# gt1/daccord

Measured on AMD Instinct MI355X. Metric: corrected Mbase/s (whole node), synthetic 20x PacBio piles, higher is better.
Workload: dtype u64+f64

## Files before the change

daccord_amd/csrc/fast_diag.hpp:

```cpp
#ifndef DACC_FAST_DIAG_HPP
#define DACC_FAST_DIAG_HPP
#if defined(DACC_EMUL)
#include <cstdint>
#include <cstdio>
#include <cstdlib>
#include <vector>
#include <algorithm>
#endif

namespace dacc {

#if defined(DACC_EMUL)
struct FastStats { enum { N = 33 }; uint32_t v[N]; void clear() { for ( int i = 0; i < N; ++i ) v[i] = 0; } void mx(int i, uint32_t x) { if ( x > v[i] ) v[i] = x; } void add(int i, uint32_t x) { v[i] += x; } };
static FastStats g_fstats;
static inline void fstats_dump(int const tier)
{
	static FILE * sf = 0; static bool tried = false;
	if ( !tried ) { tried = true; char const * fn = getenv("DACC_EMUL_STATS"); if ( fn ) sf = fopen(fn,"w"); }
	if ( sf ) { fprintf(sf,"%d",tier); for ( int i = 0; i < FastStats::N; ++i ) fprintf(sf," %u",g_fstats.v[i]); fprintf(sf,"\n"); fflush(sf); }
}
static inline FILE * ftrav_file() { static FILE * f = 0; static bool tried = false; if ( !tried ) { tried = true; char const * fn = getenv("DACC_EMUL_TRAV"); if ( fn ) f = fopen(fn,"w"); } return f; }
#define FSTAT_MX(i,x) g_fstats.mx(i,x)
#define FSTAT_ADD(i,x) g_fstats.add(i,x)
struct FeasIters { std::vector<uint32_t> it, ln; void clear() { it.clear(); ln.clear(); } };
static FeasIters g_feasit;
static inline void feasit_dump()
{
	static FILE * f = 0; static bool tried = false;
	if ( !tried ) { tried = true; char const * fn = getenv("DACC_EMUL_FEAS"); if ( fn ) f = fopen(fn,"w"); }
	if ( !f ) { g_feasit.clear(); return; }
	std::vector<uint32_t> const & it = g_feasit.it; std::vector<uint32_t> const & ln = g_feasit.ln;
	uint64_t tot = 0, lock = 0, locksorted = 0;
	for ( size_t i = 0; i < it.size(); ++i ) tot += it[i];
	for ( size_t i = 0; i < it.size(); i += 64 ) { uint32_t m = 0; for ( size_t q = i; q < it.size() && q < i+64; ++q ) m = std::max(m,it[q]); lock += m; }
	std::vector< std::pair<uint32_t,uint32_t> > P; for ( size_t i = 0; i < it.size(); ++i ) P.push_back(std::make_pair(ln[i],it[i]));
	std::stable_sort(P.begin(),P.end(),[](std::pair<uint32_t,uint32_t> const & a, std::pair<uint32_t,uint32_t> const & b){ return a.first > b.first; });
	for ( size_t i = 0; i < P.size(); i += 64 ) { uint32_t m = 0; for ( size_t q = i; q < P.size() && q < i+64; ++q ) m = std::max(m,P[q].second); locksorted += m; }
	uint64_t lockcls = 0;
	{
		std::vector< std::pair<uint32_t,uint32_t> > Q; for ( size_t i = 0; i < it.size(); ++i ) { uint32_t c = 0; while ( (2u<<c) <= ln[i] ) ++c; Q.push_back(std::make_pair(c,it[i])); }
		std::stable_sort(Q.begin(),Q.end(),[](std::pair<uint32_t,uint32_t> const & a, std::pair<uint32_t,uint32_t> const & b){ return a.first > b.first; });
		for ( size_t i = 0; i < Q.size(); i += 64 ) { uint32_t m = 0; for ( size_t q = i; q < Q.size() && q < i+64; ++q ) m = std::max(m,Q[q].second); lockcls += m; }
	}
	fprintf(f,"%zu %llu %llu %llu %llu\n",it.size(),(unsigned long long)tot,(unsigned long long)lock,(unsigned long long)locksorted,(unsigned long long)lockcls);
	g_feasit.clear();
}
static inline bool feasit_on() { static int on = -1; if ( on < 0 ) on = getenv("DACC_EMUL_FEAS") ? 1 : 0; return on == 1; }
#define FEAS_ITERS(t,len,n) { if ( feasit_on() && !feascount ) { g_feasit.it.push_back(n); g_feasit.ln.push_back(len); } }
#define FEAS_DUMP() { if ( feasit_on() && !feascount ) feasit_dump(); }
struct FeasCases
{
	enum { NU = 0, NCU, NTASK, EMPTY_FIRST, EMPTY_MID, EMPTY_LAST, START_AT_ROUND, START_AT_ROUND_END, SPANS_ROUNDS, ROUNDS, LENMASK, MAXLEN, AT_CLAMP, PAST_CLAMP, MULTI, FAIL0, FAIL1, FAILLAST, NODES, N };
	uint64_t v[N];
	void clear() { for ( int i = 0; i < N; ++i ) v[i] = 0; }
	template<typename PT> void units(PT W, uint32_t const nu)
	{
		clear();
		v[NU] = nu;
		uint32_t first = nu, last = 0;
		for ( uint32_t q = 0; q < nu; ++q ) if ( W[q] ) { if ( first == nu ) first = q; last = q; }
		uint64_t t = 0;
		for ( uint32_t q = 0; q < nu; ++q )
		{
			uint32_t const w = W[q];
			if ( !w ) { if ( q < first ) ++v[EMPTY_FIRST]; else if ( q > last ) ++v[EMPTY_LAST]; else ++v[EMPTY_MID]; continue; }
			++v[NCU];
			if ( t && t % 64 == 0 ) ++v[START_AT_ROUND];
			if ( t % 64 == 63 ) ++v[START_AT_ROUND_END];
			if ( t/64 != (t+w-1)/64 ) ++v[SPANS_ROUNDS];
			t += w;
		}
		v[NTASK] = t; v[ROUNDS] = (t+63)/64;
	}
	void node(uint32_t const j, uint32_t const len, uint32_t const pp, uint32_t const nrows, uint32_t const f)
	{
		++v[NODES];
		if ( j == 0 ) { v[LENMASK] |= 1ull << (len < 63 ? len : 63); if ( len > v[MAXLEN] ) v[MAXLEN] = len; }
		if ( pp+1 == nrows ) ++v[AT_CLAMP];
		if ( pp >= nrows ) ++v[PAST_CLAMP];
		if ( f > 1 ) ++v[MULTI];
	}
	void fail(uint32_t const j, uint32_t const len) { if ( j == 0 ) ++v[FAIL0]; if ( j == 1 ) ++v[FAIL1]; if ( j+1 == len && len > 2 ) ++v[FAILLAST]; }
	void dump(int const tier, uint32_t const nwF, uint32_t const nwR)
	{
		static FILE * f = 0; static bool tried = false;
		if ( !tried ) { tried = true; char const * fn = getenv("DACC_EMUL_FEASCASES"); if ( fn ) f = fopen(fn,"w"); }
		if ( !f ) return;
		fprintf(f,"%d",tier); for ( int i = 0; i < N; ++i ) fprintf(f," %llu",(unsigned long long)v[i]); fprintf(f," %u %u\n",nwF,nwR); fflush(f);
	}
};
static FeasCases g_feascases;
#define FEAS_UNITS(W,nu) { if ( lane == 0 && !feascount ) g_feascases.units(W,nu); }
#define FEAS_NODE(j,len,pp,nrows,f) { if ( !feascount ) g_feascases.node(j,len,pp,nrows,f); }
#define FEAS_FAIL(j,len) { if ( !feascount ) g_feascases.fail(j,len); }
#define FEAS_CASES_DUMP() { if ( lane == 0 && !feascount ) g_feascases.dump(int(CT::maxs),nwF,nwR); }
struct FeasNeedAudit
{
	enum { SCAP = 65536 };
	uint64_t outF[SCAP][3], outR[SCAP][3];
	uint64_t ntrav, units0, tasks0, units1, tasks1, recF, recR, probeF, probeR, linkR, insF, insL, mids, hlek, passes;
	FILE * f; bool tried;
	bool on() { if ( !tried ) { tried = true; char const * fn = getenv("DACC_EMUL_FEASNEED"); if ( fn ) f = fopen(fn,"w"); } return f != 0; }
	static void range(uint64_t * m, uint32_t const lo, uint32_t const hi) { for ( uint32_t p = lo; p < hi && p < 192u; ++p ) m[p>>6] |= 1ull << (p&63u); }
	void unit(uint32_t const s, bool const rev, uint32_t const lo0, uint32_t const hi0, uint32_t const lo1, uint32_t const hi1)
	{
		if ( !on() || s >= SCAP ) return;
		uint64_t * const m = rev ? outR[s] : outF[s];
		m[0] = m[1] = m[2] = 0; range(m,lo0,hi0);
		uint64_t k[3] = {0,0,0}; range(k,lo1,hi1); m[0] &= ~k[0]; m[1] &= ~k[1]; m[2] &= ~k[2];
		if ( hi0 > lo0 ) { ++units0; tasks0 += hi0-lo0; }
		if ( hi1 > lo1 ) { ++units1; tasks1 += hi1-lo1; }
	}
	static bool out(uint64_t const * m, uint32_t const p) { return p < 192u && ((m[p>>6] >> (p&63u)) & 1ull); }
	void probe(uint32_t const s, bool const rev, uint32_t const p) { if ( f && s < SCAP && out(rev ? outR[s] : outF[s],p) ) ++(rev ? probeR : probeF); }
	void link(uint32_t const a, uint32_t const b) { if ( f && a < SCAP && b < SCAP && ((outR[a][0]|outR[a][1]|outR[a][2]) || (outR[b][0]|outR[b][1]|outR[b][2])) ) ++linkR; }
	void dump()
	{
		if ( !f ) return;
		rewind(f);
		fprintf(f,"%llu %llu %llu %llu %llu %llu %llu %llu %llu %llu %llu %llu %llu %llu %llu\n",(unsigned long long)ntrav,(unsigned long long)units0,(unsigned long long)tasks0,(unsigned long long)units1,(unsigned long long)tasks1,
			(unsigned long long)recF,(unsigned long long)recR,(unsigned long long)probeF,(unsigned long long)probeR,(unsigned long long)linkR,
			(unsigned long long)insF,(unsigned long long)insL,(unsigned long long)mids,(unsigned long long)hlek,(unsigned long long)passes);
		fflush(f);
	}
	~FeasNeedAudit() { dump(); }
};
static FeasNeedAudit g_feasneed;
#define FEAS_NEED_UNIT(s,rev,lo0,hi0,lo1,hi1) { if ( !feascount ) g_feasneed.unit(s,rev,lo0,hi0,lo1,hi1); }
#define FEAS_NEED_PROBE(s,rev,p) g_feasneed.probe(s,rev,p);
#define FEAS_NEED_LINK(a,b) g_feasneed.link(a,b);
#define FEAS_OVER() { if ( !feascount ) over(128); }
#define FEAS_NEED_PASS() { if ( lane == 0 ) ++g_feasneed.passes; }
#define FEAS_NEED_DUMP() { if ( lane == 0 && !feascount && g_feasneed.on() ) { FeasNeedAudit & A_ = g_feasneed; ++A_.ntrav; A_.recF += nwF; A_.recR += nwR; A_.mids += nmid; A_.hlek += (H <= static_cast<int64_t>(k)); \
	for ( uint32_t c_ = 0; c_ < nF; ++c_ ) A_.insF += (L.fnode()[c_] != 0xFFFF && L.parF()[c_] != SNONE); for ( uint32_t c_ = 0; c_ < nL; ++c_ ) A_.insL += (L.lnode()[c_] != 0xFFFF && L.parL()[c_] != SNONE); A_.dump(); } }
#else
#define FEAS_ITERS(t,len,n)
#define FEAS_DUMP()
#define FEAS_UNITS(W,nu)
#define FEAS_NODE(j,len,pp,nrows,f)
#define FEAS_FAIL(j,len)
#define FEAS_CASES_DUMP()
#define FEAS_NEED_UNIT(s,rev,lo0,hi0,lo1,hi1)
#define FEAS_NEED_PROBE(s,rev,p)
#define FEAS_NEED_LINK(a,b)
#define FEAS_NEED_DUMP()
#define FEAS_NEED_PASS()
#define FEAS_OVER() over(128);
#define FSTAT_MX(i,x)
#define FSTAT_ADD(i,x)
#endif
}
#endif
```

daccord_amd/csrc/fast_layout.hpp:

```cpp
#ifndef DACC_FAST_LAYOUT_HPP
#define DACC_FAST_LAYOUT_HPP
#include "wave.hpp"
#include "dev_types.hpp"
#include "tier_pipeline.hpp"
#include "fast_tiers.hpp"

namespace dacc {

struct FSI { uint64_t w; uint16_t left, right, current, path; };
struct FCC { uint64_t w; uint32_t o, l; };

HDEV constexpr uint32_t fcpow2(uint32_t v) { uint32_t p = 1; while ( p < v ) p <<= 1; return p; }
HDEV constexpr uint32_t fcmax(uint32_t a, uint32_t b) { return a > b ? a : b; }
template<bool W, typename A, typename B> struct FWideSel { typedef A type; };
template<typename A, typename B> struct FWideSel<false,A,B> { typedef B type; };

#define FLD(name,type,count,start) \
	static constexpr uint32_t o_##name = (start); \
	static constexpr uint32_t e_##name = (o_##name + static_cast<uint32_t>(sizeof(type))*static_cast<uint32_t>(count) + 7u) & ~7u; \
	HDEV LDSQ type * name() const { return reinterpret_cast<LDSQ type *>(base + o_##name); }

template<typename CT, bool GW = (CT::gw != 0)> struct FastLds;

template<typename CT>
struct FastLds<CT,false>
{
	LDSQ uint8_t * base;
	static constexpr uint32_t keycap = fcpow2(CT::maxs < 2 ? 2 : CT::maxs);
	typedef uint16_t toff_t; static constexpr bool wides = false, xwides = false, ywides = false, hranges = false; static constexpr uint32_t fqmax = 255u, icap = CT::precap;
	static_assert(CT::maxs <= 256,"the legacy layout has 8 bit node frequencies and string ids");
	static_assert((CT::precap & (CT::precap-1)) == 0,"precap must be a power of two: the bitonic sorts pad to one");
	static_assert(sizeof(typename CT::id_t) > 1 || (CT::fcap <= 256 && CT::rccap <= 256),"pool slots are recorded as id_t (pout)");
	static_assert(CT::blcap <= (FastRows3<CT>::value ? 192u : 128u) && (CT::blcap & 7) == 0,"base length buckets: two 64 bit occupancy words (three in the tier of w = 128, FastRows3), cleared 8 at a time");
	static_assert(CT::lstr == 64 || CT::lstr == 128 || CT::lstr == 256,"string stride: one, two or four 64 bit words per pattern mask");
	static constexpr uint32_t pw = CT::lstr/64;
	static constexpr uint32_t maxlen = CT::lstr < 256u ? static_cast<uint32_t>(CT::lstr) : 255u;
	static constexpr uint32_t maskrows = 64u, supcap = static_cast<uint32_t>(FSUPCAP);
	typedef uint8_t sid_t;
	static_assert(sizeof(typename CT::sid_t) == 1,"16 bit stretch ids need the gw layout");
	FLD(str,uint8_t,CT::maxs*CT::lstr,0)
	FLD(slen,uint8_t,CT::maxs,e_str)
	FLD(peq,uint64_t,CT::maxs*4*pw,e_slen)
	FLD(ipos,uint8_t,CT::precap,e_peq)
	FLD(irpos,uint8_t,CT::precap,e_ipos)
	FLD(nv,uint32_t,CT::ncap,e_irpos)
	FLD(nps,uint16_t,CT::ncap+1,e_nv)
	FLD(nfreq,uint8_t,CT::ncap,e_nps)
	FLD(succ0,uint16_t,CT::ncap,e_nfreq)
	FLD(sinfo,uint16_t,CT::ncap,e_succ0)
	FLD(npred,uint8_t,CT::ncap,e_sinfo)
	FLD(nrange,uint32_t,CT::ncap,e_npred)
	FLD(mfirst,uint64_t,keycap,e_nrange)
	FLD(mlast,uint64_t,keycap,e_mfirst)
	FLD(suplo8,uint8_t,FSUPCAP,e_mlast)
	FLD(suphi8,uint8_t,FSUPCAP,e_suplo8)
	FLD(vrem,uint8_t,8,e_suphi8)
	FLD(vadd,uint8_t,8,e_vrem)
	FLD(vapos,uint8_t,8,e_vadd)
	FLD(vfn,uint16_t,8,e_vapos)
	FLD(vln,uint16_t,8,e_vfn)
	FLD(sstack,uint16_t,3*24,e_vln)
	FLD(chain,uint8_t,64,e_sstack)
	FLD(midpar,uint16_t,8,e_chain)
	FLD(midA,uint8_t,8,e_midpar)
	FLD(midB,uint8_t,8,e_midA)
	static constexpr uint32_t ubase = e_midB;
	FLD(pre,uint64_t,CT::precap,ubase)
	FLD(lastk,uint64_t,keycap,e_pre)
	static constexpr uint32_t uA = e_lastk;
	FLD(sfirst,uint16_t,CT::scap,ubase)
	FLD(slast,uint16_t,CT::scap,e_sfirst)
	FLD(sslen,uint16_t,CT::scap,e_slast)
	FLD(slink,uint16_t,CT::scap,e_sslen)
	FLD(maskF,uint64_t,CT::scap,e_slink)
	FLD(maskR,uint64_t,CT::scap,e_maskF)
	FLD(woffF,uint16_t,CT::scap,e_maskR)
	FLD(woffR,uint16_t,CT::scap,e_woffF)
	FLD(links,uint16_t,CT::lcap,e_woffR)
	FLD(wF_lo,uint32_t,CT::wcap,e_links)
	FLD(wF1_lo,uint32_t,CT::wcap,e_wF_lo)
	FLD(wFl_lo,uint32_t,CT::wcap,e_wF1_lo)
	FLD(wR_lo,uint32_t,CT::wcap,e_wFl_lo)
	FLD(wR1_lo,uint32_t,CT::wcap,e_wR_lo)
	FLD(wF_hi,uint16_t,CT::wcap,e_wR1_lo)
	FLD(wR_hi,uint16_t,CT::wcap,e_wF_hi)
	FLD(wF1_hi,uint8_t,CT::wcap,e_wR_hi)
	FLD(wFl_hi,uint8_t,CT::wcap,e_wF1_hi)
	FLD(wR1_hi,uint8_t,CT::wcap,e_wFl_hi)
	FLD(lhead,uint8_t,CT::ncap,e_wR1_hi)
	FLD(lord,uint32_t,CT::scap,e_lhead)
	FLD(ppos,uint8_t,CT::scap,e_lord)
	FLD(fkmer,uint32_t,CT::fnc,e_ppos)
	FLD(lkmer,uint32_t,CT::fnc,e_fkmer)
	FLD(fnode,uint16_t,CT::fnc,e_lkmer)
	FLD(lnode,uint16_t,CT::fnc,e_fnode)
	FLD(parF,uint8_t,CT::fnc,e_lnode)
	FLD(posF,uint8_t,CT::fnc,e_parF)
	FLD(parL,uint8_t,CT::fnc,e_posF)
	FLD(posL,uint8_t,CT::fnc,e_parL)
	FLD(pieF,uint8_t,CT::fnc,e_posL)
	FLD(pieL,uint8_t,CT::fnc,e_pieF)
	static constexpr uint32_t consmax = MAXCONS;
	static_assert(CT::wide == 0,"the wide tier needs the gw layout");
	FLD(bestL,uint8_t,MAXCONS,e_pieL)
	FLD(cdh,FCC,16,e_bestL)
	static_assert(uA <= o_cdh,"the model table copy (from o_cdh on) is loaded for gap filling while the instance array is live");
	FLD(cseq,uint8_t,18*CT::seqcap,e_cdh)
	FLD(ch,FCC,16,e_cseq)
	FLD(acc,FCC,16,e_ch)
	FLD(accerr,uint32_t,16,e_acc)
	FLD(canderr,uint8_t,16*CT::maxs,e_accerr)
	FLD(consL,uint8_t,16*CT::consrow,e_canderr)
	static constexpr uint32_t lscrbytes = static_cast<uint32_t>(CT::lscrids)*static_cast<uint32_t>(sizeof(typename CT::id_t));
	FLD(lscr,uint8_t,lscrbytes,e_cseq)
	FLD(siq,FSI,CT::siqcap,e_cseq)
	static_assert(sizeof(FSI)*CT::siqcap <= lscrbytes,"the serial score interval heap shares the lane scratch");
	static constexpr uint32_t pbase = fcmax(e_consL,e_lscr);
	FLD(rc_w,uint64_t,CT::rccap,pbase)
	FLD(rc_parent,typename CT::id_t,CT::rccap,e_rc_w)
	FLD(rc_stretch,uint8_t,CT::rccap,e_rc_parent)
	FLD(rc_pos,uint8_t,CT::rccap,e_rc_stretch)
	FLD(rc_len,uint8_t,CT::rccap,e_rc_pos)
	FLD(rc_baselen,uint8_t,CT::rccap,e_rc_len)
	FLD(rc_acc,typename CT::id_t,CT::rccap,e_rc_baselen)
	FLD(rc_ord,typename CT::id_t,CT::rccap,e_rc_acc)
	FLD(rc_arw,typename CT::id_t,CT::rccap,e_rc_ord)
	FLD(rc_sbl,uint8_t,CT::rccap,e_rc_arw)
	FLD(rc_front,uint32_t,CT::rccap,e_rc_sbl)
	FLD(rbase,uint16_t,CT::fnc+1,e_rc_front)
	FLD(rn,uint16_t,CT::fnc+1,e_rbase)
	FLD(rmaxw,uint64_t,CT::fnc+1,e_rn)
	FLD(rtmask,uint64_t,CT::fnc+1,e_rmaxw)
	FLD(rfmask,uint64_t,CT::fnc+1,e_rtmask)
	FLD(f_w,uint64_t,CT::fcap,e_rfmask)
	FLD(f_parent,typename CT::id_t,CT::fcap,e_f_w)
	FLD(f_stretch,uint8_t,CT::fcap,e_f_parent)
	FLD(f_pos,uint8_t,CT::fcap,e_f_stretch)
	FLD(f_baselen,uint8_t,CT::fcap,e_f_pos)
	FLD(f_len,uint8_t,CT::fcap,e_f_baselen)
	FLD(fp_id,typename CT::id_t,CT::fcap,e_f_len)
	FLD(fp_cl,uint8_t,CT::fcap,e_fp_id)
	FLD(fp_front,uint32_t,CT::fcap,e_fp_cl)
	FLD(fp_adj,uint64_t,CT::fcap,e_fp_front)
	FLD(fchb,uint8_t,8*CT::fnw*(CT::fnc+1),e_fp_adj)
	FLD(fnp,uint16_t,CT::fnc+1,e_fchb)
	FLD(ffm,uint64_t,CT::fnc+1,e_fnp)
	FLD(ftm,uint64_t,CT::fnc+1,e_ffm)
	FLD(fmx,uint64_t,CT::fnc+1,e_ftm)
	FLD(pout,typename CT::id_t,32*32,e_fmx)
	FLD(poutn,uint8_t,64,e_pout)
	FLD(ctr,uint32_t,4,e_poutn)
	FLD(rchx,uint8_t,32,e_ctr)
	static constexpr uint32_t upool = e_rchx;
	FLD(rchb,uint8_t,(CT::fnc < 64 ? CT::fnc : 64u)*32,o_fchb)
	static_assert(e_rchb <= o_pout,"reverse chunk lists must fit the per first k-mer tables");
	FLD(tfirst,uint16_t,CT::scap,pbase)
	FLD(tlast,uint16_t,CT::scap,e_tfirst)
	FLD(tslen,uint16_t,CT::scap,e_tlast)
	FLD(tlink,uint16_t,CT::scap,e_tslen)
	FLD(skey,uint64_t,fcpow2(CT::scap),e_tlink)
	static constexpr uint32_t uraw = e_skey;
	FLD(alpv,uint64_t,MAXCONS+1,pbase)
	FLD(almv,uint64_t,MAXCONS+1,e_alpv)
	FLD(albot,uint16_t,MAXCONS+1,e_almv)
	FLD(alops,uint8_t,2*MAXCONS+2*64+8,e_albot)
	static constexpr uint32_t ualn = e_alops;
	static constexpr uint32_t uend = fcmax(fcmax(uA,uraw),fcmax(upool,ualn));
	FLD(gfbuf,uint64_t,(pbase-uA)/8,uA)
	static constexpr uint32_t gfcap = (pbase-uA)/8;
	static constexpr uint32_t taskbytes = ((2*CT::scap+2)*2 + 2*(2*CT::scap) + 15u) & ~15u;
	FLD(toff,uint16_t,2*CT::scap+2,upool-taskbytes)
	FLD(ulo,uint8_t,2*CT::scap,e_toff)
	FLD(uhi,uint8_t,2*CT::scap,e_ulo)
	FLD(tab,uint32_t,(upool-taskbytes-o_cdh)/4,o_cdh)
	static constexpr uint32_t tabcap = (upool-taskbytes-o_cdh)/4;
	HDEV static uint32_t bytes(uint32_t const, uint32_t const) { return (uend + 15u) & ~15u; }
	static_assert(6u*CT::ncap + 16u <= e_wR1_hi - o_wF_lo,"scratch tables of the stretch walk must fit the weight arrays");
	static_assert(CT::wcap*4 >= CT::ncap*2,"interior node table must fit the weight array it borrows");
	static_assert(2u*CT::ncap + CT::scap + 8u <= 4u*CT::wcap,"reachability scratch must fit the first weight array");
	HDEV LDSQ uint32_t * xcnt32() const { return reinterpret_cast<LDSQ uint32_t *>(base + o_wF_lo); }
	HDEV LDSQ uint16_t * xstep() const { return reinterpret_cast<LDSQ uint16_t *>(base + ((e_wR1_hi - 2u*CT::ncap) & ~7u)); }
	HDEV LDSQ uint16_t * xwtmp() const { return reinterpret_cast<LDSQ uint16_t *>(base + o_wF_lo); }
	static constexpr uint32_t xnslot = (((e_wR1_hi - 2u*CT::ncap) & ~7u) - o_wF_lo) / 128u;
	HDEV LDSQ uint16_t * xsid() const { return reinterpret_cast<LDSQ uint16_t *>(base + o_wR_lo); }
	HDEV LDSQ uint8_t * xspos() const { return reinterpret_cast<LDSQ uint8_t *>(base + o_wR1_lo); }
	HDEV LDSQ uint8_t * xreach() const { return reinterpret_cast<LDSQ uint8_t *>(base + o_wF_lo); }
};

template<typename CT>
struct FastLds<CT,true>
{
	LDSQ uint8_t * base;
	static constexpr uint32_t keycap = fcpow2(CT::maxs < 2 ? 2 : CT::maxs);
	static_assert(sizeof(typename CT::id_t) > 1 || (CT::fcap <= 256 && CT::rccap <= 256),"pool slots are recorded as id_t (pout)");
	static_assert(CT::blcap <= (FastRows3<CT>::value ? 192u : 128u) && (CT::blcap & 7) == 0,"base length buckets: two 64 bit occupancy words (three in the tier of w = 128, FastRows3), cleared 8 at a time");
	static_assert(CT::lstr == 64 || CT::lstr == 128 || CT::lstr == 256,"the gw layout holds strings of up to 64 bases in one word per pattern mask, of up to 128 in two (round 6), of up to 255 in four (tier 17)");
	static constexpr uint32_t pw = CT::lstr/64;
	static constexpr uint32_t maxlen = CT::lstr < 256u ? static_cast<uint32_t>(CT::lstr) : 255u;
	static constexpr bool oneslab = FastOneSlab<CT>::value != 0;
	static constexpr bool rows3 = FastRows3<CT>::value != 0;
	static_assert(!rows3 || CT::wide != 0,"three-word position masks extend the two words of a wide tier");
	static constexpr uint32_t maskrows = CT::wide ? (rows3 ? 192u : 128u) : 64u;
	typedef typename CT::sid_t sid_t;
	static constexpr bool wides = CT::maxs > 256;
	static constexpr bool xwides = CT::maxs > 1024;
	static constexpr bool ywides = CT::maxs > 2048;
	static constexpr uint32_t fqmax = xwides ? 4095u : (wides ? 1023u : 255u);
	static constexpr bool hranges = xwides || (wides && CT::wide != 0);
	static constexpr uint32_t icap = ywides ? 16u*CT::precap : (hranges ? 8u*CT::precap : (wides ? 4u*CT::precap : CT::precap));
	static constexpr bool toff32 = xwides || (wides && CT::wide != 0);
	typedef typename FWideSel<toff32,uint32_t,uint16_t>::type toff_t;
	typedef typename FWideSel<wides,uint16_t,uint8_t>::type nfreq_t;
	typedef typename FWideSel<wides,uint32_t,uint16_t>::type nps_t;
	static_assert(fqmax <= (1u << (8u*sizeof(nfreq_t))) - 1u,"a node frequency holds fqmax");
	static_assert(icap <= (sizeof(nps_t) == 2 ? 65535u : 0xFFFFFFFFu),"nps[nn] = npre <= icap must fit a first-instance offset");
	FLD(slen,uint8_t,CT::maxs,0)
	static_assert(maxlen <= 255u,"slen: a string's length is a byte");
	static constexpr uint32_t supcap = CT::wide ? static_cast<uint32_t>(FSUPCAPW) : static_cast<uint32_t>(FSUPCAP);
	FLD(suplo8,uint8_t,supcap,e_slen)
	FLD(suphi8,uint8_t,supcap,e_suplo8)
	FLD(vrem,uint8_t,8,e_suphi8)
	FLD(vadd,uint8_t,8,e_vrem)
	FLD(vapos,uint8_t,8,e_vadd)
	FLD(vfn,uint16_t,8,e_vapos)
	FLD(vln,uint16_t,8,e_vfn)
	FLD(sstack,uint16_t,3*24,e_vln)
	FLD(chain,uint8_t,64,e_sstack)
	FLD(midpar,uint16_t,8,e_chain)
	FLD(midA,uint8_t,8,e_midpar)
	FLD(midB,uint8_t,8,e_midA)
	FLD(nv,uint32_t,CT::ncap,e_midB)
	FLD(npred,sid_t,CT::ncap,e_nv)
	static constexpr uint32_t consmax = CT::wide ? (rows3 ? 192u : 128u) : static_cast<uint32_t>(MAXCONS);
	static_assert(!rows3 || 2u + 2u*(DACC_WMAX+2u) + DACC_WMAX + consmax <= static_cast<uint32_t>(WRECW),"the wide record holds the group offsets and the symbols of a window of 128 bases: one symbol per A position and at most consmax consensus symbols");
	static constexpr uint32_t alw = CT::wide ? 2u : 1u;
	FLD(bestL,uint8_t,consmax,e_npred)
	static constexpr uint32_t sbase = (e_bestL + 15u) & ~15u;
	FLD(peq,uint64_t,CT::maxs*4*pw,sbase)
	FLD(ipos,uint8_t,icap,e_peq)
	FLD(irpos,uint8_t,icap,e_ipos)
	static_assert(supcap <= 255u && maxlen <= 255u,"ipos / irpos: the position of a k-mer in its string, from either end, is stored as min(position,nsup) <= supcap in a byte");
	FLD(nps,nps_t,CT::ncap+1,e_irpos)
	FLD(nfreq,nfreq_t,CT::ncap,e_nps)
	FLD(succ0,uint16_t,CT::ncap,e_nfreq)
	FLD(sinfo,uint16_t,CT::ncap,e_succ0)
	FLD(nrange,uint32_t,CT::ncap,e_sinfo)
	FLD(mfirst,uint64_t,keycap,e_nrange)
	FLD(mlast,uint64_t,keycap,e_mfirst)
	static constexpr uint32_t send = (e_mlast + 15u) & ~15u;
	static constexpr uint32_t sbytes = send - sbase;
	FLD(rc_w,uint64_t,CT::rccap,sbase)
	FLD(rc_parent,typename CT::id_t,CT::rccap,e_rc_w)
	FLD(rc_stretch,sid_t,CT::rccap,e_rc_parent)
	FLD(rc_pos,uint8_t,CT::rccap,e_rc_stretch)
	FLD(rc_len,uint8_t,CT::rccap,e_rc_pos)
	FLD(rc_baselen,uint8_t,CT::rccap,e_rc_len)
	FLD(rc_acc,typename CT::id_t,CT::rccap,e_rc_baselen)
	FLD(rc_ord,typename CT::id_t,CT::rccap,e_rc_acc)
	FLD(rc_arw,typename CT::id_t,CT::rccap,e_rc_ord)
	FLD(rc_sbl,uint8_t,CT::rccap,e_rc_arw)
	FLD(rc_front,uint32_t,CT::rccap,e_rc_sbl)
	FLD(rbase,uint16_t,CT::fnc+1,e_rc_front)
	FLD(rn,uint16_t,CT::fnc+1,e_rbase)
	FLD(rmaxw,uint64_t,CT::fnc+1,e_rn)
	FLD(rtmask,uint64_t,CT::fnc+1,e_rmaxw)
	FLD(rfmask,uint64_t,CT::fnc+1,e_rtmask)
	FLD(f_w,uint64_t,CT::fcap,e_rfmask)
	FLD(f_parent,typename CT::id_t,CT::fcap,e_f_w)
	FLD(f_stretch,sid_t,CT::fcap,e_f_parent)
	FLD(f_pos,uint8_t,CT::fcap,e_f_stretch)
	FLD(f_baselen,uint8_t,CT::fcap,e_f_pos)
	FLD(f_len,uint8_t,CT::fcap,e_f_baselen)
	FLD(fp_id,typename CT::id_t,CT::fcap,e_f_len)
	FLD(fp_cl,uint8_t,CT::fcap,e_fp_id)
	FLD(fp_front,uint32_t,CT::fcap,e_fp_cl)
	FLD(fp_adj,uint64_t,CT::fcap,e_fp_front)
	FLD(fchb,uint8_t,8*CT::fnw*(CT::fnc+1),e_fp_adj)
	FLD(fnp,uint16_t,CT::fnc+1,e_fchb)
	FLD(ffm,uint64_t,CT::fnc+1,e_fnp)
	FLD(ftm,uint64_t,CT::fnc+1,e_ffm)
	FLD(fmx,uint64_t,CT::fnc+1,e_ftm)
	FLD(pout,typename CT::id_t,32*32,e_fmx)
	FLD(poutn,uint8_t,64,e_pout)
	FLD(ctr,uint32_t,4,e_poutn)
	FLD(rchx,uint8_t,32,e_ctr)
	static constexpr uint32_t upool = e_rchx;
	FLD(rchb,uint8_t,(CT::fnc < 64 ? CT::fnc : 64u)*32,o_fchb)
	static_assert(e_rchb <= o_pout,"reverse chunk lists must fit the per first k-mer tables");
	static constexpr uint32_t ubase = fcmax(send,(upool + 15u) & ~15u);
	FLD(pre,uint64_t,icap,ubase)
	FLD(lastk,uint64_t,keycap,e_pre)
	static constexpr uint32_t uA = e_lastk;
	FLD(sfirst,uint16_t,CT::scap,ubase)
	FLD(slast,uint16_t,CT::scap,e_sfirst)
	FLD(sslen,uint16_t,CT::scap,e_slast)
	FLD(slink,uint16_t,CT::scap,e_sslen)
	FLD(maskF,uint64_t,CT::scap,e_slink)
	FLD(maskR,uint64_t,CT::scap,e_maskF)
	FLD(maskFh,uint64_t,(CT::wide ? CT::scap : 0u),e_maskR)
	FLD(maskRh,uint64_t,(CT::wide ? CT::scap : 0u),e_maskFh)
	FLD(maskFx,uint64_t,(rows3 ? CT::scap : 0u),e_maskRh)
	FLD(maskRx,uint64_t,(rows3 ? CT::scap : 0u),e_maskFx)
	FLD(woffF,toff_t,CT::scap,e_maskRx)
	FLD(woffR,toff_t,CT::scap,e_woffF)
	static_assert(sizeof(toff_t) == 4 || CT::wcap <= 65535u,"weight offsets of 16 bits");
	FLD(links,uint16_t,CT::lcap,e_woffR)
	FLD(lhead,sid_t,CT::ncap,e_links)
	FLD(lord,uint32_t,CT::scap,e_lhead)
	FLD(ppos,sid_t,CT::scap,e_lord)
	FLD(fkmer,uint32_t,CT::fnc,e_ppos)
	FLD(lkmer,uint32_t,CT::fnc,e_fkmer)
	FLD(fnode,uint16_t,CT::fnc,e_lkmer)
	FLD(lnode,uint16_t,CT::fnc,e_fnode)
	FLD(parF,sid_t,CT::fnc,e_lnode)
	FLD(posF,uint8_t,CT::fnc,e_parF)
	FLD(parL,sid_t,CT::fnc,e_posF)
	FLD(posL,uint8_t,CT::fnc,e_parL)
	FLD(pieF,sid_t,CT::fnc,e_posL)
	FLD(pieL,sid_t,CT::fnc,e_pieF)
	static constexpr uint32_t xbase = (e_pieL + 15u) & ~15u;
	FLD(cdh,FCC,16,xbase)
	FLD(cseq,sid_t,18*CT::seqcap,e_cdh)
	FLD(ch,FCC,16,e_cseq)
	FLD(acc,FCC,16,e_ch)
	FLD(accerr,uint32_t,16,e_acc)
	FLD(canderr,uint8_t,16*CT::maxs,e_accerr)
	static_assert(fcmax(maxlen,CT::consrow) <= 255u,"canderr: the error of a candidate against one string is at most max(string,candidate), a byte");
	FLD(consL,uint8_t,16*CT::consrow,e_canderr)
	static constexpr uint32_t lscrbytes = static_cast<uint32_t>(CT::lscrids)*static_cast<uint32_t>(sizeof(typename CT::id_t));
	FLD(lscr,uint8_t,lscrbytes,e_cseq)
	FLD(siq,FSI,CT::siqcap,e_cseq)
	static_assert(sizeof(FSI)*CT::siqcap <= lscrbytes,"the serial score interval heap shares the lane scratch");
	static constexpr uint32_t alnbytes = 2u*8u*alw*(consmax+1u) + 2u*(consmax+1u) + 8u + (2u*consmax + 2u*64u + 8u) + 16u;
	static constexpr uint32_t uB = fcmax(fcmax(fcmax(fcmax(e_consL,e_lscr),xbase + 3u*CT::ncap + 16u),xbase + (2u*CT::scap+2u)*static_cast<uint32_t>(sizeof(toff_t)) + 8u + 8u*CT::scap + 16u),CT::wide ? xbase + alnbytes : 0u);
	static constexpr uint32_t xbytes = uB - xbase;
	FLD(tfirst,uint16_t,CT::scap,o_maskF)
	FLD(tlast,uint16_t,CT::scap,e_tfirst)
	FLD(tslen,uint16_t,CT::scap,e_tlast)
	FLD(tlink,uint16_t,CT::scap,e_tslen)
	FLD(skey,uint64_t,fcpow2(CT::scap),e_tlink)
	static_assert(e_skey <= o_links,"raw stretches must fit the mask / offset arrays they borrow");
	FLD(alpv,uint64_t,alw*(consmax+1),xbase)
	FLD(almv,uint64_t,alw*(consmax+1),e_alpv)
	FLD(albot,uint16_t,consmax+1,e_almv)
	FLD(alops,uint8_t,2*consmax+2*64+8,e_albot)
	static_assert(e_alops <= uB,"final alignment scratch");
	FLD(toff,toff_t,2*CT::scap+2,xbase)
	FLD(urec,uint32_t,2*CT::scap,e_toff)
	static_assert(e_urec <= uB,"feasibility tasks");
	static_assert(3u*CT::ncap + 16u <= xbytes,"predecessor counts (a byte per node) and walking table must fit the scratch");
	static_assert(3u*CT::ncap + 16u <= xbytes && 2u*CT::ncap + CT::scap + 8u <= xbytes,"interior node table / reachability scratch");
	HDEV LDSQ uint32_t * xcnt32() const { return reinterpret_cast<LDSQ uint32_t *>(base + xbase); }
	HDEV LDSQ uint16_t * xstep() const { return reinterpret_cast<LDSQ uint16_t *>(base + xbase + ((CT::ncap + 3u) & ~3u) + 8u); }
	HDEV LDSQ uint16_t * xsid() const { return reinterpret_cast<LDSQ uint16_t *>(base + xbase); }
	HDEV LDSQ uint8_t * xspos() const { return reinterpret_cast<LDSQ uint8_t *>(base + xbase + 2u*CT::ncap + 8u); }
	HDEV LDSQ uint8_t * xreach() const { return reinterpret_cast<LDSQ uint8_t *>(base + xbase); }
	FLD(pregen,uint64_t,(wides ? icap : 0u),((fcmax(uA,uB) + 15u) & ~15u))
	static constexpr uint32_t gfown = (oneslab && !wides) ? 32768u : 0u;
	FLD(gfbuf,uint64_t,(gfown ? gfown : (uB > uA ? (uB-uA)/8 : 0u)),(gfown ? ((fcmax(uA,uB) + 15u) & ~15u) : uA))
	static constexpr uint32_t gfcap = gfown ? gfown : (uB > uA ? (uB-uA)/8 : 0u);
	static constexpr uint32_t uend = wides ? e_pregen : (gfown ? e_gfbuf : fcmax(uA,uB));
	static constexpr uint32_t tabcap = 0x7FFFFFFFu;
	HDEV static uint32_t bytes(uint32_t const, uint32_t const) { return (uend + 15u) & ~15u; }
	static constexpr uint32_t recFbytes = wides ? 32u : 16u;
	static constexpr uint32_t g_wF = 0, g_wR = recFbytes*CT::wcapg, g_spill = (recFbytes+16u)*CT::wcapg, g_inst = ((g_spill + sbytes + 255u) & ~255u),
		g_bytes = g_inst + (((icap + keycap)*8u + 255u) & ~255u);
	static_assert((o_pre & 15u) == 0 && (icap & 1u) == 0 && (keycap & 1u) == 0,"instance arrays are saved 16 bytes at a time");
	static constexpr uint32_t xnslot = g_spill / 128u;
	static constexpr uint32_t g_layout = g_bytes, g_total = CT::gmem ? g_bytes + ((((uend + 15u) & ~15u) + 255u) & ~255u) : g_bytes;
	static constexpr uint32_t g_base = oneslab ? ((((uend + 15u) & ~15u) + 255u) & ~255u) : 0u;
	static_assert(!oneslab || CT::gmem != 0,"a one-slab tier is a device-memory tier");
};
#undef FLD

template<typename CT>
HDEV FastCaps fastCapsOf(uint32_t const nrows, uint32_t const nsup)
{
	FastCaps C;
	C.maxs = CT::maxs; C.precap = FastLds<CT>::icap; C.ncap = CT::ncap; C.scap = CT::scap; C.lcap = CT::lcap; C.wcap = CT::wcap; C.rccap = CT::rccap;
	C.fcap = CT::fcap; C.siqcap = CT::siqcap; C.blcap = CT::blcap;
	C.nrows = nrows; C.nsup = nsup;
	C.ldsbytes = FastLds<CT>::bytes(nrows,nsup);
	C.tabcap = FastLds<CT>::tabcap;
	if constexpr ( CT::gw != 0 ) C.gbytes = FastLds<CT>::g_total; else C.gbytes = 0;
	if constexpr ( FastOneSlab<CT>::value != 0 ) C.ldsbytes = C.gbytes;
	C.gmem = CT::gmem;
	static_assert(CT::gmem == 0 || CT::gw != 0,"a layout in device memory is the gw layout");
	return C;
}
}
#endif
```

daccord_amd/csrc/fast_window.hpp:

```cpp
#ifndef DACC_FAST_WINDOW_HPP
#define DACC_FAST_WINDOW_HPP
#include "wave.hpp"
#include "dev_types.hpp"
#include "arena.hpp"
#include "window_main.hpp"
#include "tier_pipeline.hpp"
#include "fast_tiers.hpp"
#include "fast_layout.hpp"
#include "fast_diag.hpp"
#include "emit_record.hpp"

namespace dacc {

enum { WS_RETRY = 4 };
enum { FNOPAR = 0xFF };
enum { FSEQCAP = 48 };

struct FastBatch
{
	WindowBatch W;
	FastCaps F = {};
	uint64_t const * dpsq_vst = 0;
	uint32_t * retry = 0;
	uint32_t * gearly = 0;
// ... 1587 lines not shown

	struct REnum { ChunkList<RNW> C; uint32_t nrp, narp, lastk; };
	DEV int32_t extendReversePath(REnum & R, uint32_t const parent, uint32_t const s, uint32_t const ppos, uint32_t const plen, uint64_t const pw, uint32_t const pbl, int32_t const sfo, uint64_t const wr, uint64_t const wr1)
	{
		uint32_t const slot = clEnsure<RCH>(R.C,R.nrp,L.ctr()+0,CT::rccap/RCH);
		if ( slot == ~0u ) { over(512|0x4000); return -1; }
		uint32_t const slen = L.sslen()[s];
		uint64_t weight = pw; uint32_t baselen = pbl;
		if ( plen == 0 ) { baselen = slen+k-1; weight = sfo >= 0 ? wr : 0; }
		else { baselen += slen-1; if ( sfo >= 0 ) weight += wr - wr1; }
		uint32_t const npos = ppos + slen-1;
		if ( baselen > 255 || npos > 255 || plen+1 > 255 ) { over(2048); return -1; }
		++R.nrp;
		L.rc_parent()[slot] = parent; L.rc_stretch()[slot] = s; L.rc_len()[slot] = plen+1; L.rc_pos()[slot] = npos;
		L.rc_w()[slot] = weight; L.rc_baselen()[slot] = baselen;
		return slot;
	}
	DEV uint32_t rpFront(uint32_t const id, uint32_t const lastk) const { return L.rc_len()[id] ? L.nv()[L.sfirst()[L.rc_stretch()[id]]] : lastk; }
	DEV void reverseEnumerateLane(REnum & R, LDSQ uint8_t * chunkrow, View const & V, uint32_t const lastkmer, int32_t const lastnode, int64_t const lmax, LDSQ id_t * rpst, uint32_t const rpstcap)
	{
		clInit(R.C,chunkrow); R.nrp = 0; R.narp = 0; R.lastk = lastkmer;
		uint32_t nrpst = 0;
		if ( lastnode >= 0 )
		{
			uint32_t const slot = clEnsure<RCH>(R.C,0,L.ctr()+0,CT::rccap/RCH);
			if ( slot == ~0u ) { over(512|0x4000); return; }
			R.nrp = 1;
			L.rc_parent()[slot] = 0; L.rc_stretch()[slot] = SNONE; L.rc_len()[slot] = 0; L.rc_pos()[slot] = 0; L.rc_w()[slot] = 0; L.rc_baselen()[slot] = k;
			rpst[nrpst++] = slot;
		}
		LDSQ uint64_t const * W = L.rc_w();
		SITE_T0
		while ( nrpst )
		{
			uint32_t const rp = rpst[0];
			ipop<false>(rpst,nrpst,W);
			uint32_t const bl = L.rc_baselen()[rp], ppos = L.rc_pos()[rp], plen = L.rc_len()[rp];
			uint64_t const pw = W[rp];
			SITE(17)
			if ( R.narp >= 12 )
			{
				uint32_t cnt = 0;
				for ( uint32_t i = 0; i < R.narp; ++i )
				{
					uint32_t const a = L.rc_acc()[clSlot<RCH>(R.C,i)];
					cnt += (L.rc_baselen()[a] == bl && W[a] >= pw) ? 1 : 0;
				}
				SITE(18)
				if ( cnt >= 12 ) continue;
			}
			L.rc_acc()[clSlot<RCH>(R.C,R.narp)] = rp; ++R.narp;
			if ( plen == 0 )
			{
				MIt it; byLastBegin(V,it,lastnode);
				for ( int32_t sx = byLastNext(V,it); sx >= 0; sx = byLastNext(V,it) )
				{
					int32_t const sfo = csfFind(sx,ppos);
					WR rr; rr.w = 0; rr.w1 = 0; if ( sfo >= 0 ) rr = recR(sfo);
					uint64_t const wr = rr.w;
					if ( !(sfo >= 0 && wr >= FW_THRES_05) ) continue;
					int32_t const rpe = extendReversePath(R,rp,sx,ppos,plen,pw,bl,sfo,wr,rr.w1);
					if ( rpe < 0 ) return;
					if ( nrpst >= rpstcap ) { over(512|0x8000); return; }
					ipush<false>(rpst,nrpst,static_cast<id_t>(rpe),W);
				}
				SITE(19)
			}
			else if ( static_cast<int64_t>(bl) < (lmax+1)/2 )
			{
				uint32_t const b = L.rc_stretch()[rp];
				uint32_t const bf = L.sfirst()[b];
				MIt it; byLastBegin(V,it,bf);
				for ( int32_t ax = byLastNext(V,it); ax >= 0; ax = byLastNext(V,it) )
				{
					uint32_t const a = ax;
					if ( linkOk(a,b) )
					{
						int32_t const sfo = csfFind(a,ppos);
						WR rr; rr.w = 0; rr.w1 = 0; if ( sfo >= 0 ) rr = recR(sfo);
						uint64_t const wr = rr.w;
						if ( !(sfo >= 0 && wr >= FW_THRES_05) ) continue;
						int32_t const rpe = extendReversePath(R,rp,a,ppos,plen,pw,bl,sfo,wr,rr.w1);
						if ( rpe < 0 ) return;
						if ( nrpst >= rpstcap ) { over(512|0x8000); return; }
						ipush<false>(rpst,nrpst,static_cast<id_t>(rpe),W);
					}
					SITE(20)
				}
			}
			SITE_RESET
		}
	}
	DEV bool arpLess(uint32_t const a, uint32_t const b, uint32_t const lastk) const
	{
		uint32_t const fa = rpFront(a,lastk), fb = rpFront(b,lastk);
		if ( fa != fb ) return fa < fb;
		return L.rc_baselen()[a] < L.rc_baselen()[b];
	}
	DEV void arpULI(LDSQ id_t * last, uint32_t const lk) { id_t const val = *last; LDSQ id_t * next = last-1; while ( arpLess(val,*next,lk) ) { *last = *next; last = next; --next; } *last = val; }
	DEV void arpIns(LDSQ id_t * first, LDSQ id_t * last, uint32_t const lk)
	{
		if ( first == last ) return;
		for ( LDSQ id_t * i = first+1; i != last; ++i )
		{
			if ( arpLess(*i,*first,lk) ) { id_t const val = *i; for ( LDSQ id_t * q = i; q != first; --q ) *q = *(q-1); *first = val; }
			else arpULI(i,lk);
		}
	}
	DEV void arpSort(LDSQ id_t * first, LDSQ id_t * last, uint32_t const lk)
	{
		if ( first == last ) return;
		int32_t const n = last-first;
		if ( n > 16 )
		{
			int depth = 0; { int32_t t = n; while ( t > 1 ) { t >>= 1; ++depth; } depth *= 2; }
			LDSQ uint16_t * stF = L.sstack(); LDSQ uint16_t * stL = stF+24; LDSQ uint16_t * stD = stF+48; int sp = 0;
			stF[0] = 0; stL[0] = n; stD[0] = depth; sp = 1;
			while ( sp )
			{
				--sp;
				LDSQ id_t * f = first+stF[sp]; LDSQ id_t * l = first+stL[sp]; int d = stD[sp];
				while ( l-f > 16 )
				{
					if ( d == 0 ) { over(1024); return; }
					--d;
					LDSQ id_t * mid = f + (l-f)/2; LDSQ id_t * a = f+1; LDSQ id_t * b = mid; LDSQ id_t * c = l-1;
					if ( arpLess(*a,*b,lk) )
					{
						if ( arpLess(*b,*c,lk) ) { id_t t = *f; *f = *b; *b = t; }
						else if ( arpLess(*a,*c,lk) ) { id_t t = *f; *f = *c; *c = t; }
						else { id_t t = *f; *f = *a; *a = t; }
					}
					else if ( arpLess(*a,*c,lk) ) { id_t t = *f; *f = *a; *a = t; }
					else if ( arpLess(*b,*c,lk) ) { id_t t = *f; *f = *c; *c = t; }
					else { id_t t = *f; *f = *b; *b = t; }
					LDSQ id_t * lo = f+1; LDSQ id_t * hi = l;
					while ( true )
					{
						while ( arpLess(*lo,*f,lk) ) ++lo;
						--hi;
						while ( arpLess(*f,*hi,lk) ) --hi;
						if ( !(lo < hi) ) break;
						id_t t = *lo; *lo = *hi; *hi = t;
						++lo;
					}
					if ( sp < 24 ) { stF[sp] = lo-first; stL[sp] = l-first; stD[sp] = d; ++sp; } else { over(1024); return; }
					l = lo;
				}
			}
			arpIns(first,first+16,lk);
			for ( LDSQ id_t * i = first+16; i != last; ++i ) arpULI(i,lk);
		}
		else arpIns(first,last,lk);
	}
	DEV static void arpSwapK(LDSQ id_t * I, LDSQ uint64_t * K, int32_t const a, int32_t const b) { id_t const t = I[a]; I[a] = I[b]; I[b] = t; uint64_t const u = K[a]; K[a] = K[b]; K[b] = u; }
	DEV static void arpULIK(LDSQ id_t * I, LDSQ uint64_t * K, int32_t last) { id_t const vi = I[last]; uint64_t const vk = K[last]; int32_t next = last-1; while ( vk < K[next] ) { I[last] = I[next]; K[last] = K[next]; last = next; --next; } I[last] = vi; K[last] = vk; }
	DEV static void arpInsK(LDSQ id_t * I, LDSQ uint64_t * K, int32_t const first, int32_t const last)
	{
		if ( first == last ) return;
		for ( int32_t i = first+1; i != last; ++i )
		{
			if ( K[i] < K[first] ) { id_t const vi = I[i]; uint64_t const vk = K[i]; for ( int32_t q = i; q != first; --q ) { I[q] = I[q-1]; K[q] = K[q-1]; } I[first] = vi; K[first] = vk; }
			else arpULIK(I,K,i);
		}
	}
	DEV void arpSortK(LDSQ id_t * I, LDSQ uint64_t * K, int32_t const n)
	{
		if ( n == 0 ) return;
		if ( n > 16 )
		{
			int depth = 0; { int32_t t = n; while ( t > 1 ) { t >>= 1; ++depth; } depth *= 2; }
			LDSQ uint16_t * stF = L.sstack(); LDSQ uint16_t * stL = stF+24; LDSQ uint16_t * stD = stF+48; int sp = 0;
			stF[0] = 0; stL[0] = n; stD[0] = depth; sp = 1;
			while ( sp )
			{
				--sp;
				int32_t f = stF[sp], l = stL[sp]; int d = stD[sp];
				while ( l-f > 16 )
				{
					if ( d == 0 ) { over(1024); return; }
					--d;
					int32_t const mid = f + (l-f)/2, a = f+1, b = mid, c = l-1;
					if ( K[a] < K[b] )
					{
						if ( K[b] < K[c] ) arpSwapK(I,K,f,b);
						else if ( K[a] < K[c] ) arpSwapK(I,K,f,c);
						else arpSwapK(I,K,f,a);
					}
					else if ( K[a] < K[c] ) arpSwapK(I,K,f,a);
					else if ( K[b] < K[c] ) arpSwapK(I,K,f,c);
					else arpSwapK(I,K,f,b);
					int32_t lo = f+1, hi = l;
					while ( true )
					{
						while ( K[lo] < K[f] ) ++lo;
						--hi;
						while ( K[f] < K[hi] ) --hi;
						if ( !(lo < hi) ) break;
						arpSwapK(I,K,lo,hi);
						++lo;
					}
					if ( sp < 24 ) { stF[sp] = lo; stL[sp] = l; stD[sp] = d; ++sp; } else { over(1024); return; }
					l = lo;
				}
			}
			arpInsK(I,K,0,16);
			for ( int32_t i = 16; i != n; ++i ) arpULIK(I,K,i);
		}
		else arpInsK(I,K,0,n);
	}
	DEV void reverseBlockCopy(REnum const & R, uint32_t const sbase)
	{
		for ( uint32_t i = 0; i < R.narp; ++i ) L.rc_ord()[sbase+i] = L.rc_acc()[clSlot<RCH>(R.C,i)];
	}
	template<bool WTMP = false>
	DEV void reverseBlockFinish(REnum const & R, uint32_t const sbase, uint32_t const li, int32_t const lastnode, int64_t const lmax)
	{
		uint32_t const narp = R.narp;
		LDSQ uint64_t const * W = L.rc_w();
		constexpr bool TMP = WTMP && CT::rccap <= CT::fcap;
		LDSQ uint64_t * const WT = L.f_w() + sbase;
		uint64_t rmaxw = 0, rfm = 0;
		for ( uint32_t i = 0; i < narp; ++i ) { uint64_t const w = W[L.rc_ord()[sbase+i]]; rmaxw = w > rmaxw ? w : rmaxw; }
		if constexpr ( TMP )
		{
			for ( uint32_t i = 0; i < narp; ++i ) { uint32_t const rp = L.rc_ord()[sbase+i]; WT[i] = (static_cast<uint64_t>(rpFront(rp,R.lastk)) << 8) | L.rc_baselen()[rp]; }
			arpSortK(L.rc_ord()+sbase,WT,static_cast<int32_t>(narp));
			for ( uint32_t i = 0; i < narp; ++i ) { uint64_t const key = WT[i]; L.rc_front()[sbase+i] = static_cast<uint32_t>(key >> 8); L.rc_sbl()[sbase+i] = static_cast<uint8_t>(key & 0xFF); }
			for ( uint32_t i = 0; i < narp; ++i ) WT[i] = W[L.rc_ord()[sbase+i]];
		}
		else arpSort(L.rc_ord()+sbase,L.rc_ord()+sbase+narp,R.lastk);
		uint64_t tm = lastnode >= 0 ? (1ull << (lastnode & 63)) : 0ull;
		for ( uint32_t i = 0; i < narp; ++i )
		{
			uint32_t const rp = L.rc_ord()[sbase+i];
			uint64_t const wi = W[rp];
			uint32_t r = 0;
			if constexpr ( TMP )
			{
				uint32_t j = 0;
				for ( ; j+4 <= narp; j += 4 )
				{
					uint64_t const w0 = WT[j], w1 = WT[j+1], w2 = WT[j+2], w3 = WT[j+3];
					r += (w0 < wi || (w0 == wi && j < i)) ? 1u : 0u; r += (w1 < wi || (w1 == wi && j+1 < i)) ? 1u : 0u;
					r += (w2 < wi || (w2 == wi && j+2 < i)) ? 1u : 0u; r += (w3 < wi || (w3 == wi && j+3 < i)) ? 1u : 0u;
				}
				for ( ; j < narp; ++j ) { uint64_t const wj = WT[j]; if ( wj < wi || (wj == wi && j < i) ) ++r; }
			}
			else
			for ( uint32_t j = 0; j < narp; ++j )
			{
				uint64_t const wj = W[L.rc_ord()[sbase+j]];
				if ( wj < wi || (wj == wi && j < i) ) ++r;
			}
			L.rc_arw()[sbase+i] = r;
			uint32_t fr;
			if constexpr ( TMP ) fr = L.rc_front()[sbase+i];
			else { fr = rpFront(rp,R.lastk); L.rc_front()[sbase+i] = fr; L.rc_sbl()[sbase+i] = L.rc_baselen()[rp]; }
			rfm |= 1ull << (fr & 63);
			if ( L.rc_len()[rp] && static_cast<int64_t>(L.rc_baselen()[rp]) < (lmax+1)/2 ) tm |= 1ull << (L.sfirst()[L.rc_stretch()[rp]] & 63);
		}
		L.rbase()[li] = sbase; L.rn()[li] = narp; L.rmaxw()[li] = rmaxw; L.rtmask()[li] = tm; L.rfmask()[li] = rfm;
	}
	DEV bool reverseUnaffected(uint32_t const sbase, uint32_t const nacc2, int32_t const lastnode, uint32_t const par, uint32_t const fn, int64_t const lmax) const
	{
		uint32_t const plast = L.slast()[par];
		if ( lastnode >= 0 && (static_cast<uint32_t>(lastnode) == plast || static_cast<uint32_t>(lastnode) == fn) ) return false;
		for ( uint32_t i = 0; i < nacc2; ++i )
		{
			uint32_t const rp = L.rc_ord()[sbase+i];
			if ( L.rc_len()[rp] && static_cast<int64_t>(L.rc_baselen()[rp]) < (lmax+1)/2 )
			{
				uint32_t const target = L.sfirst()[L.rc_stretch()[rp]];
				if ( target == plast || target == fn ) return false;
			}
		}
		return true;
	}

	template<bool W, int DUMMY = 0> struct FEnumHi { }; template<int DUMMY> struct FEnumHi<true,DUMMY> { uint64_t m2; };
	struct FEnum : FEnumHi<(CT::wide != 0)> { ChunkList<FNW> C; uint32_t np, nfpop; uint64_t fmaxw, ffm, m0, m1; };
	enum : uint32_t { FBLMAX = CT::wide ? 191u : 127u };
	DEV static void fblSet(FEnum & F, uint32_t const nbl)
	{
		if constexpr ( CT::wide != 0 )
		{
			uint64_t const b = 1ull << (nbl & 63u); uint32_t const wd = nbl >> 6;
			F.m0 |= wd == 0 ? b : 0ull; F.m1 |= wd == 1 ? b : 0ull; F.m2 |= wd == 2 ? b : 0ull;
		}
	}
	DEV static bool fblAny(FEnum const & F) { if constexpr ( CT::wide != 0 ) return (F.m0 | F.m1 | F.m2) != 0; else return (F.m0 | F.m1) != 0; }
	DEV static uint32_t fblPop(FEnum & F)
	{
		if constexpr ( CT::wide == 0 ) return 0;
		else
		{
			uint32_t const wd = F.m0 ? 0u : (F.m1 ? 1u : 2u);
			uint64_t const m = wd == 0 ? F.m0 : (wd == 1 ? F.m1 : F.m2);
			uint64_t const c = m & (m-1);
			F.m0 = wd == 0 ? c : F.m0; F.m1 = wd == 1 ? c : F.m1; F.m2 = wd == 2 ? c : F.m2;
			return 64u*wd + static_cast<uint32_t>(__builtin_ctzll(m));
		}
	}
	DEV int32_t extendPath(FEnum & F, uint32_t const parent, uint32_t const s, uint32_t const ppos, uint32_t const plen, uint64_t const pw, uint32_t const pbl,
		int32_t const sfo, uint64_t const wf, uint64_t const wf1, uint32_t & npos, uint32_t & nbl, uint64_t & nw)
	{
		uint32_t const slot = clEnsure<FCH>(F.C,F.np,L.ctr()+1,CT::fcap/FCH);
		if ( slot == ~0u ) { over(512|0x10000); return -1; }
		uint32_t const slen = L.sslen()[s];
		uint64_t weight = pw; uint32_t baselen = pbl;
		if ( plen == 0 ) { baselen = slen+k-1; weight = sfo >= 0 ? wf : 0; }
		else { baselen += slen-1; if ( sfo >= 0 ) weight += wf - wf1; }
		npos = ppos + (slen-1); nbl = baselen; nw = weight;
		if ( baselen > FBLMAX || npos > 255 || plen+1 > 255 ) { over(2048); return -1; }
		++F.np;
		L.f_parent()[slot] = parent; L.f_stretch()[slot] = s; L.f_len()[slot] = plen+1; L.f_pos()[slot] = npos;
		L.f_w()[slot] = weight; L.f_baselen()[slot] = baselen;
		return slot;
	}
	DEV void forwardEnumerateLane(FEnum & F, LDSQ uint8_t * chunkrow, View const & V, int32_t const firstnode, int64_t const lmax, LDSQ id_t * hp)
	{
		clInit(F.C,chunkrow); F.np = 0; F.nfpop = 0; F.fmaxw = 0; F.ffm = 0; F.m0 = 0; F.m1 = 0; if constexpr ( CT::wide != 0 ) F.m2 = 0;
		if ( firstnode < 0 ) return;
		PROFX_T0
		SITE_T0
		{
			MIt it; byFirstBegin(V,it,firstnode);
			for ( int32_t sx = byFirstNext(V,it); sx >= 0; sx = byFirstNext(V,it) )
			{
				int32_t const sfo = sfFind(sx,0);
				uint64_t const wf = sfo >= 0 ? wuF(sfo) : 0;
				uint32_t npos, nbl; uint64_t nw;
				int32_t const id = extendPath(F,0,sx,0,0,0,0,sfo,wf,0,npos,nbl,nw);
				if ( id < 0 ) return;
				if constexpr ( CT::wide == 0 ) { if ( nbl < 64 ) F.m0 |= 1ull << nbl; else F.m1 |= 1ull << (nbl-64); } else fblSet(F,nbl);
			}
		}
		LDSQ uint64_t const * W = L.f_w();
		SITE(11)
		while ( fblAny(F) )
		{
			uint32_t zz;
			if constexpr ( CT::wide == 0 )
			{
				zz = F.m0 ? static_cast<uint32_t>(__builtin_ctzll(F.m0)) : 64u + static_cast<uint32_t>(__builtin_ctzll(F.m1));
				if ( zz < 64 ) F.m0 &= F.m0-1; else F.m1 &= F.m1-1;
			}
			else zz = fblPop(F);
			uint32_t hn = 0;
			for ( uint32_t i0 = 0; i0 < F.np; i0 += 64 )
			{
				uint64_t mem = 0;
				uint32_t const ie = (F.np-i0 < 64) ? (F.np-i0) : 64u;
				static_assert(FCH % 4 == 0,"entries per chunk");
				for ( uint32_t i = 0; i < ie; i += 4 )
				{
					uint32_t const slot = clSlot<FCH>(F.C,i0+i);
					uint32_t const b4 = *reinterpret_cast<LDSQ uint32_t const *>(L.f_baselen() + slot);
					#pragma unroll
					for ( uint32_t u = 0; u < 4; ++u ) if ( i+u < ie ) mem |= static_cast<uint64_t>(((b4 >> (8*u)) & 0xFF) == zz) << (i+u);
				}
				SITE(12)
				while ( mem )
				{
					uint32_t const i = __builtin_ctzll(mem); mem &= mem-1;
					uint32_t const e = clSlot<FCH>(F.C,i0+i);
					if ( hn == 12 )
					{
						if ( W[e] > W[hp[0]] ) { ipop<true>(hp,hn,W); ipush<true>(hp,hn,static_cast<id_t>(e),W); }
					}
					else ipush<true>(hp,hn,static_cast<id_t>(e),W);
				}
				SITE(13)
			}
			PROFX(19)
			while ( hn )
			{
				uint32_t const path = hp[0];
				ipop<true>(hp,hn,W);
				uint32_t const ps = L.f_stretch()[path], ppos = L.f_pos()[path], plen = L.f_len()[path], pbl = zz;
				uint64_t const pw = W[path];
				uint32_t const lastn = L.slast()[ps];
				SITE(14)
				{
					int32_t const psfo = sfFind(ps,ppos - (L.sslen()[ps]-1));
					uint32_t const pfront = L.nv()[lastn];
					uint32_t const o = clSlot<FCH>(F.C,F.nfpop);
					L.fp_id()[o] = path; L.fp_front()[o] = pfront; L.fp_cl()[o] = ppos; F.ffm |= 1ull << (pfront & 63);
					L.fp_adj()[o] = psfo >= 0 ? (pw - recF(psfo).wl) : pw;
					if ( pw > F.fmaxw ) F.fmaxw = pw;
					++F.nfpop;
				}
				SITE(15)
				if ( pbl < k || ( static_cast<int64_t>(pbl-k) < ((lmax+1)/2) ) )
				{
					MIt it; byFirstBegin(V,it,lastn);
					for ( int32_t sx = byFirstNext(V,it); sx >= 0; sx = byFirstNext(V,it) )
					{
						uint32_t const s = sx;
						int32_t const sfo = sfFind(s,ppos);
						WF fr; fr.w = 0; fr.w1 = 0; fr.wl = 0; if ( sfo >= 0 ) fr = recF(sfo);
						uint64_t const eweight = fr.w;
						if ( eweight >= FW_THRES_01 )
						{
							uint32_t npos, nbl; uint64_t nw;
							int32_t const ep = extendPath(F,path,s,ppos,plen,pw,pbl,sfo,eweight,fr.w1,npos,nbl,nw);
							if ( ep < 0 ) return;
							if ( nw >= FW_THRES_01 && static_cast<int64_t>(npos) + k <= lmax )
							{
								if constexpr ( CT::wide == 0 ) { if ( nbl < 64 ) F.m0 |= 1ull << nbl; else F.m1 |= 1ull << (nbl-64); } else fblSet(F,nbl);
							}
							else --F.np;
						}
						SITE(16)
					}
				}
				SITE_RESET
			}
			SITE_RESET
			PROFX(20)
		}
	}
	DEV void forwardTreeFinish(FEnum const & F, uint32_t const fi, int32_t const firstnode, int64_t const lmax)
	{
		uint64_t m = firstnode >= 0 ? (1ull << (firstnode & 63)) : 0ull;
		for ( uint32_t i = 0; i < F.nfpop; ++i )
		{
			uint32_t const path = L.fp_id()[clSlot<FCH>(F.C,i)];
			uint32_t const pbl = L.f_baselen()[path];
			if ( pbl < k || ( static_cast<int64_t>(pbl-k) < ((lmax+1)/2) ) ) m |= 1ull << (L.slast()[L.f_stretch()[path]] & 63);
		}
		L.fnp()[fi] = F.nfpop; L.ffm()[fi] = F.ffm; L.ftm()[fi] = m; L.fmx()[fi] = F.fmaxw;
	}
	DEV void forwardTreeLoad(ChunkList<FNW> & C, uint32_t const fi) const { C.ids = L.fchb() + 8*FNW*fi; C.n = 8*FNW; }
	DEV bool forwardUnaffected(ChunkList<FNW> const & C, uint32_t const nfpop, int32_t const firstnode, uint32_t const par, uint32_t const ln, int64_t const lmax) const
	{
		uint32_t const pfirst = L.sfirst()[par];
		if ( static_cast<uint32_t>(firstnode) == pfirst || static_cast<uint32_t>(firstnode) == ln ) return false;
		for ( uint32_t i = 0; i < nfpop; ++i )
		{
			uint32_t const path = L.fp_id()[clSlot<FCH>(C,i)];
			uint32_t const pbl = L.f_baselen()[path];
			if ( pbl < k || ( static_cast<int64_t>(pbl-k) < ((lmax+1)/2) ) )
			{
				uint32_t const target = L.slast()[L.f_stretch()[path]];
				if ( target == pfirst || target == ln ) return false;
			}
		}
		return true;
	}

	enum : uint32_t { FSEQCAP = CT::seqcap, CONSROW = CT::consrow };
	static_assert(CONSROW <= FastLds<CT>::consmax && (CONSROW & 7u) == 0,"rows of the decoded candidates: read as 64 bit words");
	uint32_t cfree;
	DEV uint32_t buildSeq(uint32_t const path, uint32_t const rp, LDSQ sid_t * dst, uint32_t & conslen)
	{
		uint32_t const nf = L.f_len()[path], nr = L.rc_len()[rp];
		if ( nf + nr > FSEQCAP ) { over(4096); return ~0u; }
		conslen = static_cast<uint32_t>(L.f_pos()[path]) + k + L.rc_pos()[rp];
		if ( conslen > CONSROW ) { over(4096); return ~0u; }
		uint32_t qf = path, qr = rp;
		uint32_t const ns = nf > nr ? nf : nr;
		for ( uint32_t t = 0; t < ns; ++t )
		{
			if ( t < nf ) { dst[nf-1-t] = L.f_stretch()[qf]; qf = L.f_parent()[qf]; }
			if ( t < nr ) { dst[nf+t] = L.rc_stretch()[qr]; qr = L.rc_parent()[qr]; }
		}
		return nf+nr;
	}
	DEV uint32_t decodeSeq(LDSQ sid_t const * seq, uint32_t const n, LDSQ uint8_t * dst) const
	{
		uint32_t o = 0;
		uint32_t const firstv = L.nv()[L.sfirst()[seq[0]]];
		for ( uint32_t i = 0; i < k; ++i ) dst[o++] = (firstv >> (2*(k-1-i))) & 3;
		for ( uint32_t ii = 0; ii < n; ++ii )
		{
			uint32_t const s = seq[ii]; LDSQ uint16_t const * Lk = L.links() + L.slink()[s];
			uint32_t const len = L.sslen()[s];
			for ( uint32_t j = 1; j < len; ++j ) dst[o++] = L.nv()[Lk[j]] & 3;
		}
		return o;
	}
	DEV bool scoreInterval(uint32_t const sbase, uint32_t const nacc2, uint32_t const front, int64_t const candlen, int64_t const lmin, int64_t const lmax,
		uint32_t & sub, uint32_t & sup, uint32_t & mi) const
	{
		uint32_t lo = 0, hi = nacc2;
		while ( lo < hi ) { uint32_t const mid = (lo+hi)>>1; if ( L.rc_front()[sbase+mid] < front ) lo = mid+1; else hi = mid; }
		uint32_t e = lo;
		while ( e < nacc2 && L.rc_front()[sbase+e] == front ) ++e;
		if ( e == lo ) return false;
		int64_t bllo = lmin + static_cast<int64_t>(k) - candlen; if ( bllo < 0 ) bllo = 0;
		int64_t blhi = lmax + static_cast<int64_t>(k) - candlen; if ( blhi < 0 ) blhi = 0;
		uint32_t const bllo16 = static_cast<uint16_t>(bllo), blhi16 = static_cast<uint16_t>(blhi);
		sub = lo;
		while ( sub < e && L.rc_sbl()[sbase+sub] < bllo16 ) ++sub;
		sup = sub;
		while ( sup < e && !(blhi16 < L.rc_sbl()[sbase+sup]) ) ++sup;
		if ( sub == sup ) return false;
		mi = sub; uint32_t mr = L.rc_arw()[sbase+sub];
		for ( uint32_t i = sub+1; i < sup; ++i ) { uint32_t const r = L.rc_arw()[sbase+i]; if ( r > mr ) { mi = i; mr = r; } }
		return true;
	}
	DEV bool scoreNext(uint32_t const sbase, uint32_t const left, uint32_t const right, uint32_t const current, uint32_t & bi) const
	{
		uint32_t const v = L.rc_arw()[sbase+current];
		if ( !v ) return false;
		bool found = false; uint32_t bu = 0;
		for ( uint32_t i = left; i < right; ++i )
		{
			uint32_t const r = L.rc_arw()[sbase+i];
			if ( r <= v-1 && (!found || r > bu) ) { found = true; bu = r; bi = i; }
		}
		return found;
	}
	enum : uint32_t { UNMAT = 0x80000000u };
	uint32_t pvpath, pvrp, pvcl, pvnf;
	DEV bool seqEqual(uint32_t pa, uint32_t ra, uint32_t na, uint32_t pb, uint32_t rb, uint32_t nb)
	{
		if ( na > nb ) { uint32_t t = pa; pa = pb; pb = t; t = ra; ra = rb; rb = t; t = na; na = nb; nb = t; }
		uint32_t const d = nb - na;
		if ( static_cast<uint32_t>(L.rc_len()[ra]) < d ) return false;
		LDSQ sid_t * mid = L.cseq() + 16*FSEQCAP;
		uint32_t qr = ra;
		for ( uint32_t t = 0; t < d; ++t ) { mid[t] = L.rc_stretch()[qr]; qr = L.rc_parent()[qr]; }
		if ( qr != rb ) return false;
		uint32_t qf = pb;
		for ( uint32_t t = 0; t < d; ++t )
		{
			if ( L.f_stretch()[qf] != mid[d-1-t] ) return false;
			qf = L.f_parent()[qf];
		}
		return qf == pa;
	}
	DEV bool offerCandidate(uint64_t const weight, uint32_t const path, uint32_t const rp, uint32_t & pn)
	{
		FSTAT_ADD(18,1);
		SITE_T0
		if ( ncdh == 16 ) { uint32_t const to = L.cdh()[0].o, tl = L.cdh()[0].l; if ( !(tl & UNMAT) ) cfree |= 1u << to; spop<FCC,true>(L.cdh(),ncdh); SITE(5) }
		uint32_t const nf = L.f_len()[path], nr = L.rc_len()[rp];
		uint32_t const conslen = static_cast<uint32_t>(L.f_pos()[path]) + k + L.rc_pos()[rp];
		if ( nf + nr > FSEQCAP || conslen > CONSROW ) { over(4096); return false; }
		uint32_t const n = nf+nr;
		SITE(6)
		if ( n == pn && conslen == pvcl && path != pvpath && rp != pvrp && nf != pvnf )
		{
			bool const same = seqEqual(path,rp,nf,pvpath,pvrp,pvnf);
			SITE(7)
			if ( same ) return true;
		}
		pn = n; pvpath = path; pvrp = rp; pvcl = conslen; pvnf = nf;
		FCC cc; cc.w = weight; cc.o = path | (rp << 16); cc.l = n | (conslen<<8) | UNMAT;
		FSTAT_ADD(19,1);
		spush<FCC,true>(L.cdh(),ncdh,cc);
		SITE(8)
		return true;
	}
	DEV void materializeKept()
	{
		wv_sync();
		uint32_t const n = wv_bcast(ncdh,0);
		if ( !n ) return;
		uint32_t const cf = wv_bcast(cfree,0);
		uint32_t taken = 0, done = 0;
		for ( uint32_t c0 = 0; c0 < n; c0 += WSZ )
		{
			uint32_t const c = c0 + lane;
			FCC e; e.w = 0; e.o = 0; e.l = 0;
			if ( c < n ) e = ldget(L.cdh()+c);
			bool const um = c < n && (e.l & UNMAT) != 0;
			uint32_t tot; uint32_t const rank = done + wv_scan_flag(um,tot);
			done += tot;
			if ( um )
			{
				uint32_t m = cf; for ( uint32_t i = 0; i < rank; ++i ) m &= m-1;
				uint32_t const slot = __builtin_ctz(m);
				uint32_t cl;
				buildSeq(e.o & 0xFFFFu,e.o >> 16,L.cseq() + FSEQCAP*slot,cl);
				e.o = slot; e.l &= ~static_cast<uint32_t>(UNMAT); ldput(L.cdh()+c,e);
				taken |= 1u << slot;
			}
		}
		taken = wv_or(taken);
		if ( lane == 0 ) cfree &= ~taken;
		wv_sync();
	}
	DEV void materializeSerial(uint32_t const f0, uint32_t const r0)
	{
		for ( uint32_t c = 0; c < ncdh; ++c )
		{
			uint32_t const l = L.cdh()[c].l;
			if ( !(l & UNMAT) ) continue;
			uint32_t const o = L.cdh()[c].o, pa = o & 0xFFFFu, ra = o >> 16;
			if ( pa < f0 && ra < r0 ) continue;
			uint32_t const slot = __builtin_ctz(cfree); cfree &= cfree-1;
			uint32_t cl;
			buildSeq(pa,ra,L.cseq() + FSEQCAP*slot,cl);
			L.cdh()[c].o = slot; L.cdh()[c].l = l & ~static_cast<uint32_t>(UNMAT);
		}
	}
	DEV void combinePair(ChunkList<FNW> const & FC, uint32_t const nfpop, uint32_t const sbase, uint32_t const nacc2, uint64_t const rfm, int64_t const lmin, int64_t const lmax, uint32_t const maxfullpath,
		uint32_t const skip = 0, uint32_t pn = ~0u)
	{
		nsiq = 0;
		if ( !skip ) { pvpath = pvrp = pvnf = 0; pvcl = ~0u; }
		for ( uint32_t pi = 0; pi < nfpop; ++pi )
		{
			uint32_t const o = clSlot<FCH>(FC,pi);
			uint32_t const front = L.fp_front()[o];
			if ( !((rfm >> (front & 63)) & 1) ) continue;
			uint32_t sub, sup, mi;
			if ( scoreInterval(sbase,nacc2,front,static_cast<int64_t>(L.fp_cl()[o]) + k,lmin,lmax,sub,sup,mi) )
			{
				if ( nsiq >= CT::siqcap ) { over(512|0x40000); return; }
				FSI si; si.left = sub; si.right = sup; si.current = mi; si.path = pi; si.w = L.fp_adj()[o] + L.rc_w()[L.rc_ord()[sbase+mi]];
				spush<FSI,false>(L.siq(),nsiq,si);
			}
		}
		for ( uint32_t numfullpath = 0; nsiq && numfullpath < maxfullpath; ++numfullpath )
		{
			FSI const si = ldget(L.siq());
			if ( numfullpath >= skip && ncdh == 16 && si.w <= L.cdh()[0].w ) break;
			spop<FSI,false>(L.siq(),nsiq);
			uint32_t bi;
			if ( scoreNext(sbase,si.left,si.right,si.current,bi) )
			{
				FSI sic = si; sic.current = bi; sic.w = L.fp_adj()[clSlot<FCH>(FC,si.path)] + L.rc_w()[L.rc_ord()[sbase+bi]];
				if ( nsiq >= CT::siqcap ) { over(512|0x40000); return; }
				spush<FSI,false>(L.siq(),nsiq,sic);
			}
			if ( numfullpath < skip ) continue;
			if ( !offerCandidate(si.w,L.fp_id()[clSlot<FCH>(FC,si.path)],L.rc_ord()[sbase+si.current],pn) ) return;
		}
	}
	struct PSI { id_t path, current, left, right; };
	enum { PSIQ = CT::psiq, POUTE = 8 };
	static constexpr id_t PSENT = static_cast<id_t>(~static_cast<id_t>(0));
	static_assert(sizeof(id_t) > 1 || 8u*FNW*FCH < 255u,"the end mark of a lane's interval heap must not be a forward pop index");
	bool lscrdirty;
	DEV uint64_t psiW(PSI const & e, ChunkList<FNW> const & FC, uint32_t const sbase) const { return L.fp_adj()[clSlot<FCH>(FC,e.path)] + L.rc_w()[L.rc_ord()[sbase+e.current]]; }
	DEV uint32_t combineLane(ChunkList<FNW> const & FC, uint32_t const nfpop, uint32_t const sbase, uint32_t const nacc2, uint64_t const rfm, int64_t const lmin, int64_t const lmax,
		uint32_t const maxfullpath, LDSQ PSI * H, LDSQ id_t * out, bool const prune, uint64_t const T0)
	{
		uint32_t n = 0;
		SITE_T0
		for ( uint32_t pi = 0; pi < nfpop; ++pi )
		{
			uint32_t const o = clSlot<FCH>(FC,pi);
			uint32_t const front = L.fp_front()[o];
			if ( !((rfm >> (front & 63)) & 1) ) continue;
			uint32_t sub, sup, mi;
			if ( scoreInterval(sbase,nacc2,front,static_cast<int64_t>(L.fp_cl()[o]) + k,lmin,lmax,sub,sup,mi) )
			{
				if ( n >= PSIQ || sup > 255 && sizeof(id_t) == 1 ) return 0xFF;
				PSI e; e.path = pi; e.current = mi; e.left = sub; e.right = sup;
				uint32_t i = n++; H[i] = e;
				uint64_t const we = psiW(e,FC,sbase);
				while ( i )
				{
					uint32_t const p = (i-1)>>1;
					PSI const ep = H[p];
					if ( we > psiW(ep,FC,sbase) ) { H[i] = ep; H[p] = e; i = p; }
					else break;
				}
			}
		}
		FSTAT_ADD(25,1); FSTAT_ADD(26,n > 8 ? 1u : 0u); FSTAT_ADD(27,n > 10 ? 1u : 0u); FSTAT_ADD(28,n > 12 ? 1u : 0u); FSTAT_ADD(29,n > 16 ? 1u : 0u); FSTAT_MX(30,n);
		SITE(1)
		return combineLanePops(FC,sbase,n,maxfullpath,H,out,prune,T0);
	}
	DEV uint32_t combineLanePops(ChunkList<FNW> const & FC, uint32_t const sbase, uint32_t n, uint32_t const maxfullpath, LDSQ PSI * H, LDSQ id_t * out, bool const prune, uint64_t const T0)
	{
		SITE_T0
		uint32_t cnt = 0;
		for ( uint32_t numfullpath = 0; n && numfullpath < maxfullpath; ++numfullpath )
		{
			PSI const top = H[0];
			if ( prune && psiW(top,FC,sbase) <= T0 ) { if ( n < PSIQ ) H[n].path = PSENT; return cnt | 0x20; }
			if ( cnt == POUTE ) { if ( n < PSIQ ) H[n].path = PSENT; return cnt | 0x10; }
			{
				--n; PSI const last = H[n]; H[0] = last;
				uint32_t i = 0, r;
				while ( (r = 2*i+2) < n )
				{
					uint32_t const m = psiW(H[r-1],FC,sbase) > psiW(H[r],FC,sbase) ? (r-1) : r;
					PSI const em = H[m], ei = H[i];
					if ( psiW(ei,FC,sbase) > psiW(em,FC,sbase) ) break;
					H[i] = em; H[m] = ei; i = m;
				}
				if ( r >= n )
				{
					uint32_t const l = 2*i+1;
					if ( l < n ) { PSI const el = H[l], ei = H[i]; if ( !(psiW(ei,FC,sbase) > psiW(el,FC,sbase)) ) { H[i] = el; H[l] = ei; } }
				}
			}
			uint32_t bi;
			if ( scoreNext(sbase,top.left,top.right,top.current,bi) )
			{
				PSI e = top; e.current = bi;
				uint32_t i = n++; H[i] = e;
				uint64_t const we = psiW(e,FC,sbase);
				while ( i )
				{
					uint32_t const p = (i-1)>>1;
					PSI const ep = H[p];
					if ( we > psiW(ep,FC,sbase) ) { H[i] = ep; H[p] = e; i = p; }
					else break;
				}
			}
			out[2*cnt] = static_cast<id_t>(clSlot<FCH>(FC,top.path)); out[2*cnt+1] = L.rc_ord()[sbase+top.current]; ++cnt;
			SITE(2)
		}
		return cnt;
	}
	DEV uint32_t matchPops(ChunkList<FNW> const & FC, uint32_t const nfpop, uint64_t const rfm, LDSQ PSI * H) const
	{
		uint32_t nm = 0;
		for ( uint32_t pi = 0; pi < nfpop; ++pi )
		{
			uint32_t const front = L.fp_front()[clSlot<FCH>(FC,pi)];
			if ( !((rfm >> (front & 63)) & 1) ) continue;
			if ( nm < PSIQ ) H[nm].path = static_cast<id_t>(pi);
			++nm;
		}
		return nm;
	}
	DEV bool intervalTask(ChunkList<FNW> const & FC, uint32_t const sbase, uint32_t const nacc2, int64_t const lmin, int64_t const lmax, LDSQ PSI * e) const
	{
		uint32_t const pi = e->path;
		uint32_t const o = clSlot<FCH>(FC,pi);
		uint32_t sub, sup, mi;
		if ( scoreInterval(sbase,nacc2,L.fp_front()[o],static_cast<int64_t>(L.fp_cl()[o]) + k,lmin,lmax,sub,sup,mi) )
		{
			if ( sup > 255 && sizeof(id_t) == 1 ) return false;
			PSI v; v.path = static_cast<id_t>(pi); v.current = static_cast<id_t>(mi); v.left = static_cast<id_t>(sub); v.right = static_cast<id_t>(sup);
			*e = v;
		}
		else e->path = PSENT;
		return true;
	}
	DEV uint32_t heapOfList(ChunkList<FNW> const & FC, uint32_t const sbase, LDSQ PSI * H, uint32_t const nm) const
	{
		uint32_t n = 0;
		for ( uint32_t j = 0; j < nm; ++j )
		{
			PSI const e = H[j];
			if ( e.path == PSENT ) continue;
			uint32_t i = n++; H[i] = e;
			uint64_t const we = psiW(e,FC,sbase);
			while ( i )
			{
				uint32_t const p = (i-1)>>1;
				PSI const ep = H[p];
				if ( we > psiW(ep,FC,sbase) ) { H[i] = ep; H[p] = e; i = p; }
				else break;
			}
		}
		return n;
	}
	DEV bool replayPair(ChunkList<FNW> const & FC, uint32_t const sbase, LDSQ id_t const * out, uint32_t const cnt, uint32_t & pn)
	{
		pn = ~0u; pvpath = pvrp = pvnf = 0; pvcl = ~0u;
		FSTAT_ADD(16,1); FSTAT_ADD(17,cnt);
		SITE_T0
		for ( uint32_t e = 0; e < cnt; ++e )
		{
			uint32_t const o = out[2*e];
			uint32_t const rp = out[2*e+1];
			uint64_t const w = L.fp_adj()[o] + L.rc_w()[rp];
			if ( ncdh == 16 && w <= L.cdh()[0].w ) { if ( e == 0 ) FSTAT_ADD(20,1); SITE(4) return false; }
			uint32_t const fid = L.fp_id()[o];
			SITE(4)
			if ( !offerCandidate(w,fid,rp,pn) ) return false;
			SITE_RESET
		}
		return true;
	}

	DEV void continueLane(ChunkList<FNW> const & FC, uint32_t const sbase, LDSQ PSI * H, uint32_t const cnt, uint32_t pn)
	{
		uint32_t n = 0;
		while ( n < PSIQ && H[n].path != PSENT ) ++n;
		for ( uint32_t numfullpath = cnt; n && numfullpath < 16; ++numfullpath )
		{
			PSI const top = H[0];
			uint64_t const wtop = psiW(top,FC,sbase);
			if ( ncdh == 16 && wtop <= L.cdh()[0].w ) break;
			{
				--n; PSI const last = H[n]; H[0] = last;
				uint32_t i = 0, r;
				while ( (r = 2*i+2) < n )
				{
					uint32_t const m = psiW(H[r-1],FC,sbase) > psiW(H[r],FC,sbase) ? (r-1) : r;
					PSI const em = H[m], ei = H[i];
					if ( psiW(ei,FC,sbase) > psiW(em,FC,sbase) ) break;
					H[i] = em; H[m] = ei; i = m;
				}
				if ( r >= n )
				{
					uint32_t const l = 2*i+1;
					if ( l < n ) { PSI const el = H[l], ei = H[i]; if ( !(psiW(ei,FC,sbase) > psiW(el,FC,sbase)) ) { H[i] = el; H[l] = ei; } }
				}
			}
			uint32_t bi;
			if ( scoreNext(sbase,top.left,top.right,top.current,bi) )
			{
				PSI e = top; e.current = bi;
				uint32_t i = n++; H[i] = e;
				uint64_t const we = psiW(e,FC,sbase);
				while ( i )
				{
					uint32_t const p = (i-1)>>1;
					PSI const ep = H[p];
					if ( we > psiW(ep,FC,sbase) ) { H[i] = ep; H[p] = e; i = p; }
					else break;
				}
			}
			if ( !offerCandidate(wtop,L.fp_id()[clSlot<FCH>(FC,top.path)],L.rc_ord()[sbase+top.current],pn) ) return;
		}
	}

	DEV uint32_t myersDistance(uint32_t const j, LDSQ uint8_t const * text, uint32_t const n) const
	{
		uint32_t const m = L.slen()[j];
		if ( m == 0 ) return n;
		if constexpr ( FastLds<CT>::pw > 2 ) return myersDistanceN(j,text,n,m);
		else {
		if ( FastLds<CT>::pw == 2 ) return myersDistance2(j,text,n,m);
		LDSQ uint64_t const * PEQ = L.peq() + 4*j;
		uint64_t const e0 = PEQ[0], e1 = PEQ[1], e2 = PEQ[2], e3 = PEQ[3];
		LDSQ uint64_t const * T8 = reinterpret_cast<LDSQ uint64_t const *>(text);
		uint32_t score = m;
		uint64_t Pv = ~0ull, Mv = 0;
		uint64_t const top = 1ull<<(m-1);
		uint64_t w = n ? T8[0] : 0ull;
		for ( uint32_t c0 = 0; c0 < n; c0 += 8 )
		{
			uint64_t const wn = (c0+8 < n) ? T8[(c0>>3)+1] : 0ull;
			uint32_t const cnt = (n-c0 < 8) ? (n-c0) : 8u;
			for ( uint32_t u = 0; u < cnt; ++u )
			{
				uint32_t const ch = static_cast<uint32_t>(w >> (8*u)) & 3u;
				uint64_t const Eq = (ch & 2) ? ((ch & 1) ? e3 : e2) : ((ch & 1) ? e1 : e0);
				uint64_t const Xv = Eq | Mv;
				uint64_t const Xh = (((Eq & Pv) + Pv) ^ Pv) | Eq;
				uint64_t Ph = Mv | ~(Xh | Pv);
				uint64_t Mh = Pv & Xh;
				if ( Ph & top ) ++score; else if ( Mh & top ) --score;
				Ph = (Ph<<1) | 1ull; Mh <<= 1;
				Pv = Mh | ~(Xv | Ph);
				Mv = Ph & Xv;
			}
			w = wn;
		}
		return score;
		}
	}
	DEV uint32_t myersDistance2(uint32_t const j, LDSQ uint8_t const * text, uint32_t const n, uint32_t const m) const
	{
		LDSQ uint64_t const * PEQ = L.peq() + 8*j;
		uint64_t const a0 = PEQ[0], a1 = PEQ[1], c0_ = PEQ[2], c1_ = PEQ[3], g0 = PEQ[4], g1 = PEQ[5], t0 = PEQ[6], t1 = PEQ[7];
		LDSQ uint64_t const * T8 = reinterpret_cast<LDSQ uint64_t const *>(text);
		bool const two = m > 64;
		uint64_t const top = two ? (1ull<<(m-65)) : (1ull<<(m-1));
		uint32_t score = m;
		uint64_t Pv0 = ~0ull, Mv0 = 0, Pv1 = ~0ull, Mv1 = 0;
		uint64_t w = n ? T8[0] : 0ull;
		for ( uint32_t c0 = 0; c0 < n; c0 += 8 )
		{
			uint64_t const wn = (c0+8 < n) ? T8[(c0>>3)+1] : 0ull;
			uint32_t const cnt = (n-c0 < 8) ? (n-c0) : 8u;
			for ( uint32_t u = 0; u < cnt; ++u )
			{
				uint32_t const ch = static_cast<uint32_t>(w >> (8*u)) & 3u;
				uint64_t const Eq0 = (ch & 2) ? ((ch & 1) ? t0 : g0) : ((ch & 1) ? c0_ : a0);
				uint64_t const Eq1 = (ch & 2) ? ((ch & 1) ? t1 : g1) : ((ch & 1) ? c1_ : a1);
				uint64_t const Xv0 = Eq0 | Mv0;
				uint64_t const Xh0 = (((Eq0 & Pv0) + Pv0) ^ Pv0) | Eq0;
				uint64_t Ph0 = Mv0 | ~(Xh0 | Pv0);
				uint64_t Mh0 = Pv0 & Xh0;
				uint64_t const phc = Ph0>>63, mhc = Mh0>>63;
				if ( !two ) { if ( Ph0 & top ) ++score; else if ( Mh0 & top ) --score; }
				Ph0 = (Ph0<<1) | 1ull; Mh0 <<= 1;
				Pv0 = Mh0 | ~(Xv0 | Ph0);
				Mv0 = Ph0 & Xv0;
				if ( two )
				{
					uint64_t const Eq1c = Eq1 | mhc;
					uint64_t const Xv1 = Eq1 | Mv1;
					uint64_t const Xh1 = (((Eq1c & Pv1) + Pv1) ^ Pv1) | Eq1c;
					uint64_t Ph1 = Mv1 | ~(Xh1 | Pv1);
					uint64_t Mh1 = Pv1 & Xh1;
					if ( Ph1 & top ) ++score; else if ( Mh1 & top ) --score;
					Ph1 = (Ph1<<1) | phc; Mh1 = (Mh1<<1) | mhc;
					Pv1 = Mh1 | ~(Xv1 | Ph1);
					Mv1 = Ph1 & Xv1;
				}
			}
			w = wn;
		}
		return score;
	}
	DEV uint32_t myersDistanceN(uint32_t const j, LDSQ uint8_t const * text, uint32_t const n, uint32_t const m) const
	{
		enum { PW = FastLds<CT>::pw };
		LDSQ uint64_t const * PEQ = L.peq() + 4*PW*j;
		uint64_t E0[PW], E1[PW], E2[PW], E3[PW], Pv[PW], Mv[PW];
		#pragma unroll
		for ( uint32_t b = 0; b < PW; ++b ) { E0[b] = PEQ[b]; E1[b] = PEQ[PW+b]; E2[b] = PEQ[2*PW+b]; E3[b] = PEQ[3*PW+b]; Pv[b] = ~0ull; Mv[b] = 0; }
		LDSQ uint64_t const * T8 = reinterpret_cast<LDSQ uint64_t const *>(text);
		uint32_t const lastw = (m-1) >> 6;
		uint64_t const top = 1ull << ((m-1) & 63u);
		uint32_t score = m;
		uint64_t w = n ? T8[0] : 0ull;
		for ( uint32_t c0 = 0; c0 < n; c0 += 8 )
		{
			uint64_t const wn = (c0+8 < n) ? T8[(c0>>3)+1] : 0ull;
			uint32_t const cnt = (n-c0 < 8) ? (n-c0) : 8u;
			for ( uint32_t u = 0; u < cnt; ++u )
			{
				uint32_t const ch = static_cast<uint32_t>(w >> (8*u)) & 3u;
				uint64_t const s0 = ch == 0 ? ~0ull : 0ull, s1 = ch == 1 ? ~0ull : 0ull, s2 = ch == 2 ? ~0ull : 0ull, s3 = ch == 3 ? ~0ull : 0ull;
				uint64_t phc = 1ull, mhc = 0ull;
				#pragma unroll
				for ( uint32_t b = 0; b < PW; ++b )
					if ( b <= lastw )
					{
						uint64_t const Eq = (E0[b] & s0) | (E1[b] & s1) | (E2[b] & s2) | (E3[b] & s3);
						uint64_t const Eqc = Eq | mhc;
						uint64_t const Xv = Eq | Mv[b];
						uint64_t const Xh = (((Eqc & Pv[b]) + Pv[b]) ^ Pv[b]) | Eqc;
						uint64_t Ph = Mv[b] | ~(Xh | Pv[b]);
						uint64_t Mh = Pv[b] & Xh;
						if ( b == lastw ) { if ( Ph & top ) ++score; else if ( Mh & top ) --score; }
						uint64_t const pho = Ph>>63, mho = Mh>>63;
						Ph = (Ph<<1) | phc; Mh = (Mh<<1) | mhc;
						Pv[b] = Mh | ~(Xv | Ph);
						Mv[b] = Ph & Xv;
						phc = pho; mhc = mho;
					}
			}
			w = wn;
		}
		return score;
	}
	DEV void buildPeq()
	{
		if constexpr ( GW ) return;
		else
		for ( uint32_t j = lane; j < mao; j += WSZ )
		{
			uint32_t const m = L.slen()[j];
			LDSQ uint8_t const * s = L.str() + j*CT::lstr;
			enum { PW = FastLds<CT>::pw };
			#pragma unroll
			for ( uint32_t wq = 0; wq < PW; ++wq )
			{
				uint64_t e0 = 0, e1 = 0, e2 = 0, e3 = 0;
				uint32_t const lo = 64*wq, hi = m < lo+64 ? m : lo+64;
				for ( uint32_t i = lo; i < hi; ++i )
				{
					uint32_t const c = s[i]; uint64_t const b = 1ull<<(i-lo);
					e0 |= (c == 0) ? b : 0; e1 |= (c == 1) ? b : 0; e2 |= (c == 2) ? b : 0; e3 |= (c == 3) ? b : 0;
				}
				L.peq()[4*PW*j+0*PW+wq] = e0; L.peq()[4*PW*j+1*PW+wq] = e1; L.peq()[4*PW*j+2*PW+wq] = e2; L.peq()[4*PW*j+3*PW+wq] = e3;
			}
		}
		wv_sync();
	}

	bool sfresh, sdirty;
	DEV void spillS()
	{
		if constexpr ( GW )
		{
			typedef FastLds<CT> LL;
			constexpr uint32_t plen = ((LL::upool - LL::sbase + 15u) & ~15u) < LL::sbytes ? ((LL::upool - LL::sbase + 15u) & ~15u) : LL::sbytes;
			constexpr uint32_t si0 = (LL::o_sinfo - LL::sbase) & ~15u, si1 = ((LL::e_sinfo - LL::sbase + 15u) & ~15u) < plen ? ((LL::e_sinfo - LL::sbase + 15u) & ~15u) : plen;
			LDSQ G4 const * const src = reinterpret_cast<LDSQ G4 const *>(L.base + LL::sbase);
			G4 * const dst = reinterpret_cast<G4 *>(gslab + LL::g_spill);
			wv_sync();
			if ( sfresh ) { for ( uint32_t i = lane; i < plen/16u; i += WSZ ) dst[i] = src[i]; }
			else if ( sdirty && si0 < si1 ) { for ( uint32_t i = si0/16u + lane; i < si1/16u; i += WSZ ) dst[i] = src[i]; }
			sfresh = false; sdirty = false;
			wv_sync();
		}
	}
	DEV void saveInstances()
	{
		if constexpr ( GW )
		{
			typedef FastLds<CT> LL;
			G4 * const dst = reinterpret_cast<G4 *>(gslab + LL::g_inst);
			LDSQ G4 const * const sp = reinterpret_cast<LDSQ G4 const *>(L.pre());
			LDSQ G4 const * const sl = reinterpret_cast<LDSQ G4 const *>(L.lastk());
			for ( uint32_t i = lane; i < (npre+1)/2; i += WSZ ) dst[i] = sp[i];
			for ( uint32_t i = lane; i < (nlast+1)/2; i += WSZ ) dst[FastLds<CT>::icap/2 + i] = sl[i];
		}
	}
	DEV uint32_t saveHand(FastBatch const & FB, uint32_t hslot)
	{
		if ( hslot ) return hslot;
		if ( npre + 2u*((nlast+1)/2) + 4u > FB.handwords || npre > FB.handwords ) return 0;
		uint32_t sl = 0;
		if ( lane == 0 ) { uint32_t const q = wv_atomic_add_global(FB.handctr,1u); sl = q < FB.handcap ? q+1 : 0u; }
		sl = wv_bcast(sl,0);
		if ( !sl ) return 0;
		uint64_t * const dst = FB.hand + static_cast<uint64_t>(sl-1)*FB.handwords;
		if ( lane == 0 ) { dst[0] = npre | (static_cast<uint64_t>(nlast)<<32); dst[1] = k; }
		uint32_t const po = 2, lo = 2 + ((npre+1)&~1u);
		for ( uint32_t i = lane; i < npre; i += WSZ ) dst[po+i] = L.pre()[i];
		for ( uint32_t i = lane; i < nlast; i += WSZ ) dst[lo+i] = L.lastk()[i];
		return sl;
	}
	DEV bool loadHand(FastBatch const & FB, uint32_t const hslot)
	{
		uint64_t const * const src = FB.hand + static_cast<uint64_t>(hslot-1)*FB.handwords;
		uint64_t const h0 = src[0];
		uint32_t const n = static_cast<uint32_t>(h0), nl = static_cast<uint32_t>(h0>>32);
		if ( n > FastLds<CT>::icap || nl > FastLds<CT>::keycap || src[1] != k ) return false;
		npre = n; nlast = nl;
		FSTAT_ADD(31,1);
		uint32_t const po = 2, lo = 2 + ((n+1)&~1u);
		wv_sync();
		for ( uint32_t i = lane; i < n; i += WSZ ) L.pre()[i] = src[po+i];
		for ( uint32_t i = lane; i < nl; i += WSZ ) L.lastk()[i] = src[lo+i];
		wv_sync();
		return true;
	}
	DEV void restoreInstances()
	{
		if constexpr ( GW )
		{
			typedef FastLds<CT> LL;
			G4 const * const src = reinterpret_cast<G4 const *>(gslab + LL::g_inst);
			LDSQ G4 * const dp = reinterpret_cast<LDSQ G4 *>(L.pre());
			LDSQ G4 * const dl = reinterpret_cast<LDSQ G4 *>(L.lastk());
			wv_sync();
			for ( uint32_t i = lane; i < (npre+1)/2; i += WSZ ) dp[i] = src[i];
			for ( uint32_t i = lane; i < (nlast+1)/2; i += WSZ ) dl[i] = src[FastLds<CT>::icap/2 + i];
			wv_sync();
		}
	}
	DEV void restoreS()
	{
		if constexpr ( GW )
		{
			typedef FastLds<CT> LL;
			constexpr uint32_t plen = ((LL::upool - LL::sbase + 15u) & ~15u) < LL::sbytes ? ((LL::upool - LL::sbase + 15u) & ~15u) : LL::sbytes;
			LDSQ G4 * const dst = reinterpret_cast<LDSQ G4 *>(L.base + LL::sbase);
			G4 const * const src = reinterpret_cast<G4 const *>(gslab + LL::g_spill);
			wv_sync();
			for ( uint32_t i = lane; i < plen/16u; i += WSZ ) dst[i] = src[i];
			wv_sync();
		}
	}

	enum { NPL = 64, RPSTL = 32, PM_SKIP = 0xF0, PM_SERIAL = 0xF1, PM_EXACT = 0xE0, PM_PEND = 0x80 };
	static_assert(sizeof(PSI)*PSIQ*NPL <= FastLds<CT>::lscrbytes && 2u*POUTE*NPL <= 32u*32u,"score interval heaps and pop records of a round of pairs");
	enum : uint32_t { MIDCAP = 8 };
	uint32_t nmid, midbase;
	uint32_t nLmagic;
	DEV void pairFL(uint32_t const p, uint32_t & f, uint32_t & l) const
	{
		if ( nL <= 1 ) { f = p; l = 0; }
		else
		{
#if defined(DACC_EMUL)
			f = static_cast<uint32_t>((static_cast<uint64_t>(p) * nLmagic) >> 32);
#else
			f = __umulhi(p,nLmagic);
#endif
			l = p - f*nL;
		}
	}
	uint32_t rstop;
	uint64_t roundT0;
	uint32_t nsiq, ncdh, nacc;

	DEV void viewOfLast(View & V, uint32_t const li) const
	{
		viewClear(V);
		uint32_t const sl = L.parL()[li];
		if ( sl != SNONE ) { viewRemove(V,sl); viewAdd(V,L.pieL()[li]); viewAdd(V,L.pieL()[li]+1); }
	}
	DEV void viewOfFirst(View & V, uint32_t const fi) const
	{
		viewClear(V);
		uint32_t const sf = L.parF()[fi];
		if ( sf != SNONE ) { viewRemove(V,sf); viewAdd(V,L.pieF()[fi]); viewAdd(V,L.pieF()[fi]+1); }
	}
	DEV uint32_t classifyPair(uint32_t const fi, uint32_t const li, int64_t const lmax) const
	{
		uint32_t const sf = L.parF()[fi], sl = L.parL()[li];
		if ( sf != SNONE && sf == sl ) return 4;
		int32_t const firstnode = L.fnode()[fi] == 0xFFFF ? -1 : L.fnode()[fi];
		int32_t const lastnode = L.lnode()[li] == 0xFFFF ? -1 : L.lnode()[li];
		bool rcached, fcached;
		if ( sf == SNONE ) rcached = true;
		else
		{
			uint64_t const tm = L.rtmask()[li];
			uint32_t const fn = L.fnode()[fi];
			rcached = !((tm >> (L.slast()[sf]&63))&1) && !((tm >> (fn&63))&1);
			if ( !rcached ) rcached = reverseUnaffected(L.rbase()[li],L.rn()[li],lastnode,sf,fn,lmax);
		}
		if ( sl == SNONE ) fcached = true;
		else
		{
			uint64_t const tm = L.ftm()[fi];
			fcached = !((tm >> (L.sfirst()[sl]&63))&1) && !((tm >> (L.lnode()[li]&63))&1);
			if ( !fcached ) { ChunkList<FNW> FC; forwardTreeLoad(FC,fi); fcached = forwardUnaffected(FC,L.fnp()[fi],firstnode,sl,L.lnode()[li],lmax); }
		}
		return (rcached ? 1u : 0u) | (fcached ? 2u : 0u);
	}
	DEV uint32_t replayRound(uint32_t & q, uint32_t const n, uint32_t const p0, uint32_t const fstart, int64_t const lmin, int64_t const lmax, bool const alone, uint64_t const live)
	{
		for ( ; q < n; ++q )
		{
			uint64_t const rest = live >> q;
			if ( !rest ) { q = n; break; }
			q += static_cast<uint32_t>(__builtin_ctzll(rest));
			SITE_T0
			uint32_t const mode = L.poutn()[q];
			FSTAT_ADD(13,1);
			if ( mode == PM_SKIP ) { FSTAT_ADD(14,1); continue; }
			uint32_t const p = p0+q;
			uint32_t fi, li; pairFL(p,fi,li); fi += fstart;
			if ( mode < 0x40 || mode == PM_SERIAL )
			{
				if ( ncdh == 16 && L.fmx()[fi] + L.rmaxw()[li] <= L.cdh()[0].w ) { FSTAT_ADD(15,1); SITE(3) continue; }
				ChunkList<FNW> FC; forwardTreeLoad(FC,fi);
				SITE(3)
				if ( mode < 0x40 )
				{
					uint32_t const cnt = mode & 0x0F; uint32_t pn;
					bool const used = replayPair(FC,L.rbase()[li],L.pout() + 2*POUTE*q,cnt,pn);
					if ( flags ) return 0;
					SITE_RESET
					if ( used && ( (mode & 0x10) || ((mode & 0x20) && !(ncdh == 16 && L.cdh()[0].w >= roundT0)) ) )
					{
						pcount(21,1);
						if ( !lscrdirty ) continueLane(FC,L.rbase()[li],reinterpret_cast<LDSQ PSI *>(L.lscr()) + PSIQ*q,cnt,pn);
						else combinePair(FC,L.fnp()[fi],L.rbase()[li],L.rn()[li],L.rfmask()[li],lmin,lmax,16,cnt,pn);
						SITE(9)
					}
				}
				else { pcount(23,1); lscrdirty = true; combinePair(FC,L.fnp()[fi],L.rbase()[li],L.rn()[li],L.rfmask()[li],lmin,lmax,16); SITE(9) }
				if ( flags ) return 0;
				continue;
			}
			pcount(22,1);
			lscrdirty = true;
			bool const rcached = mode & 1, fcached = mode & 2, same = mode & 4;
			uint32_t const sf = L.parF()[fi], sl = L.parL()[li];
			int32_t const firstnode = L.fnode()[fi] == 0xFFFF ? -1 : L.fnode()[fi];
			int32_t const lastnode = L.lnode()[li] == 0xFFFF ? -1 : L.lnode()[li];
			View V; viewClear(V);
			if ( same )
			{
				uint32_t const pf = L.posF()[fi], pl = L.posL()[li];
				viewRemove(V,sf);
				if ( pf == pl ) { viewAdd(V,L.pieF()[fi]); viewAdd(V,L.pieF()[fi]+1); }
				else
				{
					uint32_t const lo = pf < pl ? pf : pl, hi = pf < pl ? pl : pf;
					uint32_t m = 0;
					while ( m+1 < nmid && !(L.midpar()[m] == sf && L.midA()[m] == lo && L.midB()[m] == hi) ) ++m;
					if ( pf < pl ) { viewAdd(V,L.pieF()[fi]); viewAdd(V,L.pieL()[li]+1); } else { viewAdd(V,L.pieL()[li]); viewAdd(V,L.pieF()[fi]+1); }
					viewAdd(V,midbase+m);
				}
			}
			else
			{
				if ( sf != SNONE ) { viewRemove(V,sf); viewAdd(V,L.pieF()[fi]); viewAdd(V,L.pieF()[fi]+1); }
				if ( sl != SNONE ) { viewRemove(V,sl); viewAdd(V,L.pieL()[li]); viewAdd(V,L.pieL()[li]+1); }
			}
			uint32_t const rsave = L.ctr()[0], fsave = L.ctr()[1];
			uint32_t sbase = L.rbase()[li], nacc2 = L.rn()[li]; uint64_t rfm = L.rfmask()[li];
			if ( !rcached )
			{
				REnum RX;
				reverseEnumerateLane(RX,L.rchx(),V,L.lkmer()[li],lastnode,lmax,reinterpret_cast<LDSQ id_t *>(L.lscr()),FastLds<CT>::lscrbytes/sizeof(id_t));
				if ( flags ) return 0;
				if ( rstop + RX.narp > CT::rccap ) { over(512|0x4000); return 0; }
				reverseBlockCopy(RX,rstop);
				reverseBlockFinish(RX,rstop,FNC,lastnode,lmax);
				if ( flags ) return 0;
				sbase = rstop; nacc2 = RX.narp; rfm = L.rfmask()[FNC];
			}
			ChunkList<FNW> FC; uint32_t nfp; uint64_t ffmx;
			if ( !fcached )
			{
				FEnum FX;
				forwardEnumerateLane(FX,L.fchb() + 8*FNW*FNC,V,firstnode,lmax,reinterpret_cast<LDSQ id_t *>(L.lscr()));
				if ( flags == (512|0x10000) && FX.np < 8*FNW*FCH && !alone )
				{
					flags = 0; L.ctr()[0] = rsave; L.ctr()[1] = fsave;
					return 2;
				}
				if ( flags ) return 0;
				FC = FX.C; nfp = FX.nfpop; ffmx = FX.ffm;
			}
			else { forwardTreeLoad(FC,fi); nfp = L.fnp()[fi]; ffmx = L.ffm()[fi]; }
			if ( rfm & ffmx ) combinePair(FC,nfp,sbase,nacc2,rfm,lmin,lmax,16);
			if ( !flags && (!rcached || !fcached) ) materializeSerial(fcached ? ~0u : fsave*FCH,rcached ? ~0u : rsave*RCH);
			L.ctr()[0] = rsave; L.ctr()[1] = fsave;
			SITE(10)
			if ( flags ) return 0;
		}
		return 0;
	}

	DEV bool traverse(int64_t const lmin, int64_t const lmax)
	{
		PROF_T0
		cfree = 0xFFFFu; ncdh = 0; nacc = 0; nwF = 0; nwR = 0; nsiq = 0; pvpath = pvrp = pvnf = 0; pvcl = ~0u;
		LEDGER_REP(5) computeBaseStretches();
		flags = wv_or(flags); if ( flags ) return false;
		PROF(*this,8)
		LEDGER_REP(6) findCandidatesAndPieces();
		flags = wv_or(flags); if ( flags ) return false;
		nLmagic = nL > 1 ? static_cast<uint32_t>(((1ull<<32) + nL - 1u) / nL) : 0u;
#if !defined(DACC_NO_REACH)
		{
			SITE_T0
			bool reach = false;
			LEDGER_REP(7) reach = pairReachable();
			SITE(23)
			if ( !reach ) { FSTAT_ADD(23,1); PROF(*this,16) return false; }
		}
#endif
		computeStretchLookups();
		makePieces();
		PROF(*this,16)
		loadTab();
		PROF(*this,17)
		LEDGER_REP(8) { nwF = 0; nwR = 0; bool const need = feasNeedOn(); if ( need ) feasDistances(); computeStretchFeasLanes(0,npool,lmax,need); }
		flags = wv_or(flags); if ( flags ) return false;
#if defined(DACC_EMUL)
		nwFall = nwF; nwRall = nwR;
		if ( ftrav_file() && feasapplied )
		{
			uint32_t const kF = nwF, kR = nwR;
			feascount = true; nwF = 0; nwR = 0; computeStretchFeasLanes(0,npool,lmax,false); feascount = false;
			nwFall = nwF; nwRall = nwR; nwF = kF; nwR = kR;
		}
#endif
		{ SITE_T0 bool const sf0_ = sfresh, sd0_ = sdirty; LEDGER_REP(9) { sfresh = sf0_; sdirty = sd0_; spillS(); } SITE(24) }
		PROF(*this,9)

		LEDGER_REP(10)
		{
		if ( lane == 0 ) { L.ctr()[0] = 0; L.ctr()[1] = 0; }
		wv_sync();
		{
			uint32_t sb = 0;
			for ( uint32_t c = 0; c < nL; c += WSZ )
			{
				uint32_t const li = c + lane;
				bool const ract = li < nL;
				REnum R; clInit(R.C,L.rchb() + 8*RNW*lane); R.nrp = 0; R.narp = 0; R.lastk = 0;
				int32_t lastnode = -1;
				View V; viewClear(V);
				bool rover = false;
				if ( ract )
				{
					viewOfLast(V,li);
					lastnode = L.lnode()[li] == 0xFFFF ? -1 : L.lnode()[li];
					reverseEnumerateLane(R,L.rchb() + 8*RNW*lane,V,L.lkmer()[li],lastnode,lmax,reinterpret_cast<LDSQ id_t *>(L.lscr()) + RPSTL*lane,RPSTL);
					if ( flags == (512|0x8000) ) { rover = true; flags = 0; }
				}
				for ( uint64_t ro = wv_ballot(rover); ro; ro &= ro-1 )
				{
					wv_sync();
					if ( lane == static_cast<int>(__builtin_ctzll(ro)) )
						reverseEnumerateLane(R,L.rchb() + 8*RNW*lane,V,L.lkmer()[li],lastnode,lmax,reinterpret_cast<LDSQ id_t *>(L.lscr()),FastLds<CT>::lscrbytes/sizeof(id_t));
				}
				wv_sync();
				flags = wv_or(flags); if ( flags ) return false;
				uint32_t tot; uint32_t const sbase = sb + wv_scan_excl(ract ? R.narp : 0u,tot);
				if ( sb + tot > CT::rccap ) { over(512|0x4000); return false; }
#if defined(DACC_EMUL)
				if ( ract ) { FILE * f = ftrav_file(); if ( f ) fprintf(f,"R %d %u %u 0\n",int(CT::maxs),R.nrp,R.narp); }
#endif
				SITE_T0
				if ( ract ) reverseBlockCopy(R,sbase);
				uint64_t big = wv_ballot(ract && R.narp > 16);
				if ( ract && R.narp <= 16 ) reverseBlockFinish<true>(R,sbase,li,lastnode,lmax);
				while ( big )
				{
					int const b = __builtin_ctzll(big); big &= big-1;
					if ( lane == b ) reverseBlockFinish<true>(R,sbase,li,lastnode,lmax);
				}
				SITE(21)
				sb += tot;
				flags = wv_or(flags); if ( flags ) return false;
			}
			rstop = sb;
		}
		wv_sync();
		}
		PROF(*this,11)

		uint32_t fstart = 0, bw = WSZ, pskip = 0;
		while ( fstart < nF )
		{
			materializeKept();
			uint32_t const fi = fstart + lane;
			bool const fact = static_cast<uint32_t>(lane) < bw && fi < nF;
			FEnum F; int32_t firstnode = -1; uint32_t fover = 0;
			LEDGER_REP(11)
			{
			if ( lane == 0 ) L.ctr()[1] = 0;
			wv_sync();
			clInit(F.C,L.fchb() + 8*FNW*(fi < nF ? fi : static_cast<uint32_t>(FNC))); F.np = 0; F.nfpop = 0; F.fmaxw = 0; F.ffm = 0; F.m0 = 0; F.m1 = 0; if constexpr ( CT::wide != 0 ) F.m2 = 0;
			firstnode = -1;
			fover = 0;
			if ( fact )
			{
				uint32_t const saved = flags; flags = 0;
				View V; viewOfFirst(V,fi);
				firstnode = L.fnode()[fi] == 0xFFFF ? -1 : L.fnode()[fi];
				forwardEnumerateLane(F,L.fchb() + 8*FNW*fi,V,firstnode,lmax,reinterpret_cast<LDSQ id_t *>(L.lscr()) + 12*lane);
				if ( flags == (512|0x10000) && F.np < 8*FNW*FCH ) { fover = 1; flags = saved; }
				else flags |= saved;
#if defined(DACC_EMUL)
				{ FILE * f = ftrav_file(); if ( f ) fprintf(f,"T %d %u %u %u\n",int(CT::maxs),F.np,F.nfpop,fover); }
#endif
			}
#if defined(DACC_LEDGER)
			wv_sync();
#endif
			}
			flags = wv_or(flags); if ( flags ) return false;
			uint64_t const fo = wv_ballot(fover);
			uint32_t nb = nF - fstart; if ( nb > bw ) nb = bw;
			if ( fo ) { uint32_t const f0 = __builtin_ctzll(fo); if ( f0 < nb ) nb = f0; }
			if ( nb == 0 )
			{
				if ( bw == 1 ) { over(512|0x10000); return false; }
				bw = 1;
				continue;
			}
			if ( fo )
			{
				if ( nb == 1 && bw != 1 ) { bw = 1; continue; }
				uint32_t mx = 0;
				if ( fact && static_cast<uint32_t>(lane) < nb ) for ( uint32_t i = 0; i < F.C.n; ++i ) { uint32_t const id = F.C.ids[i]; mx = id+1 > mx ? id+1 : mx; }
				mx = wv_max(mx);
				if ( lane == 0 ) L.ctr()[1] = mx;
				wv_sync();
			}
			bw = fo ? nb : ((2*bw < WSZ) ? 2*bw : static_cast<uint32_t>(WSZ));
			{ SITE_T0 if ( fact && static_cast<uint32_t>(lane) < nb ) forwardTreeFinish(F,fi,firstnode,lmax); SITE(22) }
			wv_sync();
			PROF(*this,10)
			if ( lane == 0 ) { pcount(26,1); pcount(25,nb*nL); }
			uint32_t const npairs = nb*nL;
			bool restart = false;
			for ( uint32_t p0 = pskip; p0 < npairs && !restart; p0 += NPL )
			{
				uint32_t const nround = (npairs-p0 < NPL) ? (npairs-p0) : static_cast<uint32_t>(NPL);
				bool const cfull = wv_bcast(ncdh == 16 ? 1u : 0u,0) != 0;
				roundT0 = cfull ? L.cdh()[0].w : 0ull;
				uint64_t live = 0;
				static_assert(NPL <= 64,"one bit per pair of a round");
				LEDGER_REP(12)
				{
				live = 0;
				LDSQ PSI * const HH = reinterpret_cast<LDSQ PSI *>(L.lscr());
				uint32_t ntask = 0;
				for ( uint32_t t0 = 0; t0 < nround; t0 += WSZ )
				{
					uint32_t const t = t0 + lane;
					uint32_t mode = PM_SKIP;
					if ( t < nround )
					{
						uint32_t const p = p0 + t;
						uint32_t pfi, pli; pairFL(p,pfi,pli); pfi += fstart;
						SITE_T0
						uint32_t const cl = classifyPair(pfi,pli,lmax);
						SITE(26)
						if ( cl != 3 ) mode = PM_EXACT | cl;
						else if ( (L.rfmask()[pli] & L.ffm()[pfi]) == 0 ) mode = PM_SKIP;
						else
						{
							ChunkList<FNW> FC; forwardTreeLoad(FC,pfi);
							uint32_t const nm = matchPops(FC,L.fnp()[pfi],L.rfmask()[pli],HH + PSIQ*t);
							if ( nm == 0 ) mode = PM_SKIP;
							else mode = PM_PEND | (nm <= PSIQ ? nm : 15u);
						}
						L.poutn()[t] = mode;
					}
					uint32_t tot; wv_scan_excl(((mode & 0xF0u) == PM_PEND && (mode & 0x0Fu) != 15u) ? (mode & 0x0Fu) : 0u,tot);
					ntask += tot;
				}
				wv_sync();
				LDSQ uint16_t * const TL = reinterpret_cast<LDSQ uint16_t *>(L.pout());
				enum : uint32_t { TLCAP = 32u*32u*static_cast<uint32_t>(sizeof(id_t))/2u };
				bool const flat = ntask != 0 && ntask <= TLCAP;
				if ( flat )
				{
					uint32_t tb = 0;
					for ( uint32_t t0 = 0; t0 < nround; t0 += WSZ )
					{
						uint32_t const t = t0 + lane;
						uint32_t const mode = t < nround ? L.poutn()[t] : static_cast<uint32_t>(PM_SKIP);
						uint32_t const nm = ((mode & 0xF0u) == PM_PEND && (mode & 0x0Fu) != 15u) ? (mode & 0x0Fu) : 0u;
						uint32_t tot; uint32_t const pre = tb + wv_scan_excl(nm,tot);
						for ( uint32_t j = 0; j < nm; ++j ) TL[pre+j] = static_cast<uint16_t>(t | (j << 6));
						tb += tot;
					}
					wv_sync();
					for ( uint32_t q0 = 0; q0 < ntask; q0 += WSZ )
					{
						uint32_t const q = q0 + lane;
						if ( q < ntask )
						{
							uint32_t const en = TL[q], t = en & 63u, j = en >> 6;
							uint32_t const p = p0 + t;
							uint32_t pfi, pli; pairFL(p,pfi,pli); pfi += fstart;
							ChunkList<FNW> FC; forwardTreeLoad(FC,pfi);
							if ( !intervalTask(FC,L.rbase()[pli],L.rn()[pli],lmin,lmax,HH + PSIQ*t + j) ) L.poutn()[t] = PM_SERIAL;
						}
					}
					wv_sync();
				}
				for ( uint32_t t = lane; t < nround; t += WSZ )
				{
					uint32_t mode = L.poutn()[t];
					if ( (mode & 0xF0u) == PM_PEND )
					{
						uint32_t const p = p0 + t;
						uint32_t pfi, pli; pairFL(p,pfi,pli); pfi += fstart;
						ChunkList<FNW> FC; forwardTreeLoad(FC,pfi);
						uint32_t cnt;
						if ( flat && (mode & 0x0Fu) != 15u )
						{
							uint32_t const n = heapOfList(FC,L.rbase()[pli],HH + PSIQ*t,mode & 0x0Fu);
							cnt = combineLanePops(FC,L.rbase()[pli],n,16,HH + PSIQ*t,L.pout() + 2*POUTE*t,cfull,roundT0);
						}
						else cnt = combineLane(FC,L.fnp()[pfi],L.rbase()[pli],L.rn()[pli],L.rfmask()[pli],lmin,lmax,16,HH + PSIQ*t,L.pout() + 2*POUTE*t,cfull,roundT0);
						mode = cnt == 0xFF ? static_cast<uint32_t>(PM_SERIAL) : (cnt ? cnt : static_cast<uint32_t>(PM_SKIP));
						L.poutn()[t] = mode;
					}
					if ( mode != PM_SKIP ) live |= 1ull << t;
				}
				live = wv_or64(live);
				wv_sync();
				}
				PROF(*this,5)
				if ( lane == 0 ) pcount(27,1);
				uint32_t q = 0;
				while ( true )
// ... 629 lines not shown
```

daccord_amd/csrc/wave.hpp:

```cpp
#ifndef DACC_WAVE_HPP
#define DACC_WAVE_HPP
#include <stdint.h>

#if defined(DACC_EMUL) && defined(DACC_EMUL_LANES) && DACC_EMUL_LANES == 64
  #define DEV inline
  #define HDEV inline
  #define WSZ 64
  #include "wave_emul64.hpp"
#elif defined(DACC_EMUL)
  #define DEV inline
  #define HDEV inline
  #define WSZ 1
  namespace dacc {
  static inline int wv_lane() { return 0; }
  static inline void wv_sync() {}
  static inline uint32_t wv_scan_excl(uint32_t v, uint32_t & total) { total = v; return 0; }
  static inline uint32_t wv_scan_flag(bool p, uint32_t & total) { total = p ? 1u : 0u; return 0; }
  static inline uint32_t wv_sum(uint32_t v) { return v; }
  static inline uint64_t wv_sum64(uint64_t v) { return v; }
  static inline uint32_t wv_max(uint32_t v) { return v; }
  static inline uint64_t wv_max64(uint64_t v) { return v; }
  static inline uint64_t wv_min64(uint64_t v) { return v; }
  static inline int wv_any(int p) { return p; }
  static inline uint32_t wv_or(uint32_t v) { return v; }
// ... 51 lines not shown
  {
	uint32_t const lo = __builtin_amdgcn_readfirstlane(static_cast<uint32_t>(v)), hi = __builtin_amdgcn_readfirstlane(static_cast<uint32_t>(v>>32));
	return (static_cast<uint64_t>(hi)<<32) | lo;
  }
  DEV uint32_t wv_sum(uint32_t v)
  {
	DACC_DPP_SCAN(v,DACC_OP_ADD,0u)
	return static_cast<uint32_t>(__builtin_amdgcn_readlane(static_cast<int>(v),63));
  }
  DEV uint64_t wv_sum64(uint64_t v)
  {
	#pragma unroll
	for ( int d = 32; d >= 1; d >>= 1 ) v += __shfl_xor(v,d,64);
	return wv_uni64(v);
  }
  DEV uint32_t wv_max(uint32_t v)
  {
	DACC_DPP_SCAN(v,DACC_OP_MAX,0u)
	return static_cast<uint32_t>(__builtin_amdgcn_readlane(static_cast<int>(v),63));
  }
  DEV uint64_t wv_max64(uint64_t v)
  {
	#pragma unroll
	for ( int d = 32; d >= 1; d >>= 1 ) { uint64_t const o = __shfl_xor(v,d,64); v = o > v ? o : v; }
	return wv_uni64(v);
  }
  DEV uint64_t wv_min64(uint64_t v)
  {
	#pragma unroll
	for ( int d = 32; d >= 1; d >>= 1 ) { uint64_t const o = __shfl_xor(v,d,64); v = o < v ? o : v; }
	return wv_uni64(v);
  }
  DEV int wv_any(int p) { return __any(p); }
  DEV uint32_t wv_or(uint32_t v)
  {
	DACC_DPP_SCAN(v,DACC_OP_OR,0u)
	return static_cast<uint32_t>(__builtin_amdgcn_readlane(static_cast<int>(v),63));
  }
  DEV uint64_t wv_or64(uint64_t v)
  {
	uint32_t lo = static_cast<uint32_t>(v), hi = static_cast<uint32_t>(v>>32);
	DACC_DPP_SCAN(lo,DACC_OP_OR,0u)
	DACC_DPP_SCAN(hi,DACC_OP_OR,0u)
	uint32_t const l = static_cast<uint32_t>(__builtin_amdgcn_readlane(static_cast<int>(lo),63)), h = static_cast<uint32_t>(__builtin_amdgcn_readlane(static_cast<int>(hi),63));
	return (static_cast<uint64_t>(h)<<32) | l;
  }
  DEV uint64_t wv_ballot(int p) { return __ballot(p); }
  DEV uint64_t wv_lanemask_lt() { return (1ull << (threadIdx.x & 63)) - 1ull; }
  DEV uint32_t wv_bcast(uint32_t v, int src) { return static_cast<uint32_t>(__builtin_amdgcn_readlane(static_cast<int>(v),__builtin_amdgcn_readfirstlane(src))); }
  DEV uint64_t wv_bcast64(uint64_t v, int src)
  {
	int const sl = __builtin_amdgcn_readfirstlane(src);
	uint32_t const lo = static_cast<uint32_t>(__builtin_amdgcn_readlane(static_cast<int>(static_cast<uint32_t>(v)),sl)), hi = static_cast<uint32_t>(__builtin_amdgcn_readlane(static_cast<int>(static_cast<uint32_t>(v>>32)),sl));
	return (static_cast<uint64_t>(hi)<<32) | lo;
  }
  DEV uint32_t wv_shfl(uint32_t v, int src) { return __shfl(v,src,64); }
  DEV uint64_t wv_shfl64(uint64_t v, int src) { return __shfl(v,src,64); }
  DEV int dacc_popc64(uint64_t v) { return __popcll(v); }
  DEV void atomicOrFlag(uint32_t * f) { atomicOr(f,1u); }
  template<typename PT> DEV uint32_t wv_atomic_add(PT p, uint32_t const v) { return __hip_atomic_fetch_add(p,v,__ATOMIC_RELAXED,__HIP_MEMORY_SCOPE_WORKGROUP); }
  DEV uint32_t wv_atomic_add_global(uint32_t * p, uint32_t const v) { return __hip_atomic_fetch_add(p,v,__ATOMIC_RELAXED,__HIP_MEMORY_SCOPE_AGENT); }
  }
#endif

#if defined(__HIP_DEVICE_COMPILE__) && defined(DACC_LAYOUT_IN_GLOBAL)
#define LDSQ __attribute__((address_space(1)))
#define GLBQ __attribute__((address_space(1)))
#elif defined(__HIP_DEVICE_COMPILE__)
#define LDSQ __attribute__((address_space(3)))
#define GLBQ __attribute__((address_space(1)))
#else
#define LDSQ
#define GLBQ
#endif

namespace dacc {

template<typename PT>
DEV void wv_bitonic_sort(PT A, uint32_t const n)
{
	int const lane = wv_lane();
	for ( uint32_t k = 2; k <= n; k <<= 1 )
		for ( uint32_t j = k>>1; j > 0; j >>= 1 )
		{
			for ( uint32_t t = lane; t < (n>>1); t += WSZ )
			{
				uint32_t const i = ((t & ~(j-1)) << 1) | (t & (j-1));
				uint32_t const l = i | j;
				uint64_t const a = A[i], b = A[l];
				bool const up = ((i & k) == 0);
				if ( (a > b) == up ) { A[i] = b; A[l] = a; }
			}
			wv_sync();
		}
}

template<typename PT>
DEV void wv_cx4(PT A, uint32_t const n, uint32_t const i0, uint32_t const l0, uint32_t const i1, uint32_t const l1,
	uint32_t const i2, uint32_t const l2, uint32_t const i3, uint32_t const l3)
{
	bool const v0 = l0 < n, v1 = l1 < n, v2 = l2 < n, v3 = l3 < n;
	uint64_t a0 = 0, b0 = 0, a1 = 0, b1 = 0, a2 = 0, b2 = 0, a3 = 0, b3 = 0;
	if ( v0 ) { a0 = A[i0]; b0 = A[l0]; }
	if ( v1 ) { a1 = A[i1]; b1 = A[l1]; }
	if ( v2 ) { a2 = A[i2]; b2 = A[l2]; }
	if ( v3 ) { a3 = A[i3]; b3 = A[l3]; }
	if ( v0 && a0 > b0 ) { A[i0] = b0; A[l0] = a0; }
	if ( v1 && a1 > b1 ) { A[i1] = b1; A[l1] = a1; }
	if ( v2 && a2 > b2 ) { A[i2] = b2; A[l2] = a2; }
	if ( v3 && a3 > b3 ) { A[i3] = b3; A[l3] = a3; }
}
template<typename PT>
DEV void wv_bitonic_sort_n(PT A, uint32_t const n)
{
	int const lane = wv_lane();
	uint32_t n2 = 1; while ( n2 < n ) n2 <<= 1;
	uint32_t const half = n2>>1;
	for ( uint32_t k = 2; k <= n2; k <<= 1 )
	{
		uint32_t const h = k>>1;
		for ( uint32_t t = lane; t < half; t += 4*WSZ )
		{
			uint32_t I[4], Lx[4];
			#pragma unroll
			for ( uint32_t u = 0; u < 4; ++u )
			{
				uint32_t const tt = t + u*WSZ;
				uint32_t const blk = tt / h, off = tt - blk*h;
				I[u] = blk*k + off; Lx[u] = (tt < half) ? (blk*k + (k-1-off)) : n;
			}
			wv_cx4(A,n,I[0],Lx[0],I[1],Lx[1],I[2],Lx[2],I[3],Lx[3]);
		}
		wv_sync();
		for ( uint32_t j = k>>2; j > 0; j >>= 1 )
		{
			for ( uint32_t t = lane; t < half; t += 4*WSZ )
			{
				uint32_t I[4], Lx[4];
				#pragma unroll
				for ( uint32_t u = 0; u < 4; ++u )
				{
					uint32_t const tt = t + u*WSZ;
					I[u] = ((tt & ~(j-1)) << 1) | (tt & (j-1)); Lx[u] = (tt < half) ? (I[u] | j) : n;
				}
				wv_cx4(A,n,I[0],Lx[0],I[1],Lx[1],I[2],Lx[2],I[3],Lx[3]);
			}
			wv_sync();
		}
	}
}

DEV void wv_bitonic_sort_idx(uint32_t * I, uint64_t const * K, uint32_t const n)
{
	int const lane = wv_lane();
	for ( uint32_t k = 2; k <= n; k <<= 1 )
		for ( uint32_t j = k>>1; j > 0; j >>= 1 )
		{
			for ( uint32_t t = lane; t < (n>>1); t += WSZ )
			{
				uint32_t const i = ((t & ~(j-1)) << 1) | (t & (j-1));
				uint32_t const l = i | j;
				uint32_t const a = I[i], b = I[l];
				bool gt;
				if ( a == 0xFFFFFFFFu ) gt = (b != 0xFFFFFFFFu);
				else if ( b == 0xFFFFFFFFu ) gt = false;
				else { uint64_t const ka = K[a], kb = K[b]; gt = (ka > kb) || (ka == kb && a > b); }
				bool const up = ((i & k) == 0);
				if ( gt == up ) { I[i] = b; I[l] = a; }
			}
			wv_sync();
		}
}

#if WSZ == 64
template<int R, int J> DEV void wv_sort_inlane(uint64_t (&v)[R], uint32_t const base, uint32_t const k)
{
	#pragma unroll
	for ( int r = 0; r < R; ++r )
		if ( (r & J) == 0 )
		{
			uint64_t const a = v[r], b = v[r|J];
			bool const up = ((base + r) & k) == 0;
			bool const sw = (a > b) == up;
			v[r] = sw ? b : a; v[r|J] = sw ? a : b;
		}
}
template<int R, typename PT>
DEV void wv_sort_regs(PT A, uint32_t const n)
{
	static_assert(R == 2 || R == 4 || R == 8 || R == 16 || R == 32,"elements per lane");
	uint32_t const lane = wv_lane(), base = lane*R;
	uint64_t v[R];
	#pragma unroll
	for ( int r = 0; r < R; ++r ) v[r] = (base + r < n) ? A[base+r] : ~0ull;
	uint32_t n2 = 2; while ( n2 < n ) n2 <<= 1;
	for ( uint32_t k = 2; k <= n2; k <<= 1 )
	{
		for ( uint32_t j = k>>1; j >= static_cast<uint32_t>(R); j >>= 1 )
		{
			uint32_t const m = j/R;
			bool const keepmin = ((lane & m) == 0) == ((base & k) == 0);
			#pragma unroll
			for ( int r = 0; r < R; ++r )
			{
				uint64_t const p = wv_shfl64(v[r],static_cast<int>(lane ^ m));
				bool const plt = p < v[r];
				v[r] = (plt == keepmin) ? p : v[r];
			}
		}
		uint32_t const h = k>>1;
		if ( R > 16 && h >= 16 ) wv_sort_inlane<R,(R > 16 ? 16 : 1)>(v,base,k);
		if ( R > 8 && h >= 8 ) wv_sort_inlane<R,(R > 8 ? 8 : 1)>(v,base,k);
		if ( R > 4 && h >= 4 ) wv_sort_inlane<R,(R > 4 ? 4 : 1)>(v,base,k);
		if ( R > 2 && h >= 2 ) wv_sort_inlane<R,(R > 2 ? 2 : 1)>(v,base,k);
		wv_sort_inlane<R,1>(v,base,k);
	}
	wv_sync();
	#pragma unroll
	for ( int r = 0; r < R; ++r ) if ( base + r < n ) A[base+r] = v[r];
	wv_sync();
}
template<int R>
DEV void wv_sort_regs_merge_steps(uint64_t (&v)[R], uint32_t const lane, uint32_t const base, uint32_t const k, uint32_t const jfirst)
{
	for ( uint32_t j = jfirst; j >= static_cast<uint32_t>(R); j >>= 1 )
	{
		uint32_t const m = j/R;
		bool const keepmin = ((lane & m) == 0) == ((base & k) == 0);
		#pragma unroll
		for ( int r = 0; r < R; ++r )
		{
			uint64_t const p = wv_shfl64(v[r],static_cast<int>(lane ^ m));
			bool const plt = p < v[r];
			v[r] = (plt == keepmin) ? p : v[r];
		}
	}
	if ( R > 16 ) wv_sort_inlane<R,(R > 16 ? 16 : 1)>(v,base,k);
	if ( R > 8 ) wv_sort_inlane<R,(R > 8 ? 8 : 1)>(v,base,k);
	if ( R > 4 ) wv_sort_inlane<R,(R > 4 ? 4 : 1)>(v,base,k);
	if ( R > 2 ) wv_sort_inlane<R,(R > 2 ? 2 : 1)>(v,base,k);
	wv_sort_inlane<R,1>(v,base,k);
}
template<typename PT>
DEV void wv_sort_two_halves(PT A, uint32_t const n)
{
	enum { R = 16, H = 64*R };
	wv_sort_regs<R>(A,H);
	wv_sort_regs<R>(A+H,n-H);
	uint32_t const lane = wv_lane(), base = lane*R;
	uint64_t v[R];
	#pragma unroll
	for ( int r = 0; r < R; ++r ) v[r] = A[base+r];
	#pragma unroll
	for ( int r = 0; r < R; ++r )
	{
		uint32_t const q = 2*H-1-(base+r);
		if ( q < n ) { uint64_t const b = A[q]; if ( v[r] > b ) { A[q] = v[r]; v[r] = b; } }
	}
	wv_sort_regs_merge_steps<R>(v,lane,base,2*H,H/2);
	wv_sync();
	#pragma unroll
	for ( int r = 0; r < R; ++r ) A[base+r] = v[r];
	#pragma unroll
	for ( int r = 0; r < R; ++r ) v[r] = (H+base+r < n) ? A[H+base+r] : ~0ull;
	wv_sort_regs_merge_steps<R>(v,lane,base,2*H,H/2);
	wv_sync();
	#pragma unroll
	for ( int r = 0; r < R; ++r ) if ( H+base+r < n ) A[H+base+r] = v[r];
	wv_sync();
}
#endif
template<uint32_t CAP, bool R32 = false, typename PT>
DEV void wv_sort_keys(PT A, uint32_t const n)
{
#if WSZ == 64
	if ( CAP <= 128 || n <= 128 ) { wv_sort_regs<2>(A,n); return; }
	if ( CAP <= 256 || n <= 256 ) { wv_sort_regs<4>(A,n); return; }
	if ( CAP <= 512 || n <= 512 ) { wv_sort_regs<8>(A,n); return; }
	if ( CAP <= 1024 || n <= 1024 ) { wv_sort_regs<16>(A,n); return; }
#if defined(DACC_SORT2H)
	if ( R32 && (CAP <= 2048 || n <= 2048) ) { wv_sort_two_halves(A,n); return; }
#else
	if ( R32 && (CAP <= 2048 || n <= 2048) ) { wv_sort_regs<32>(A,n); return; }
#endif
#endif
	wv_bitonic_sort_n(A,n);
}

HDEV uint32_t dacc_rev32(uint32_t x)
{
#if defined(__clang__)
	return __builtin_bitreverse32(x);
#else
	x = ((x >> 1) & 0x55555555u) | ((x & 0x55555555u) << 1); x = ((x >> 2) & 0x33333333u) | ((x & 0x33333333u) << 2);
	x = ((x >> 4) & 0x0F0F0F0Fu) | ((x & 0x0F0F0F0Fu) << 4); x = ((x >> 8) & 0x00FF00FFu) | ((x & 0x00FF00FFu) << 8);
	return (x >> 16) | (x << 16);
#endif
}
HDEV uint32_t dacc_spread16(uint32_t x)
{
	x &= 0xFFFFu; x = (x | (x << 8)) & 0x00FF00FFu; x = (x | (x << 4)) & 0x0F0F0F0Fu; x = (x | (x << 2)) & 0x33333333u; x = (x | (x << 1)) & 0x55555555u;
	return x;
}
HDEV uint32_t next_pow2(uint32_t v)
{
	uint32_t p = 1;
	while ( p < v ) p <<= 1;
	return p;
}

}
#endif
```

Baseline: 42.63.

## Pack forward-path entries into one word and index pop data by path slot

Forward path nodes (parent, stretch, pos, len) can be stored as a single packed 32-bit LDS word in tiers with byte-sized ids, so a node is read with one load. The fp_cl array is removed, and pop-side arrays fp_front and fp_adj are now indexed by path slot instead of pop index, so interval heaps carry path ids directly and skip the clSlot and fp_id indirection. The baselen match over four bytes uses a SWAR equality trick instead of a per-byte loop. Emulation-only trace events are added. The change trades LDS layout complexity for fewer loads and less indirection, and risks lengths above 255 or different heap sentinel semantics, since the end mark now uses right==0.

```diff
diff --git a/daccord_amd/csrc/fast_diag.hpp b/daccord_amd/csrc/fast_diag.hpp
--- a/daccord_amd/csrc/fast_diag.hpp
+++ b/daccord_amd/csrc/fast_diag.hpp
@@ -22,6 +22,7 @@
 static inline FILE * ftrav_file() { static FILE * f = 0; static bool tried = false; if ( !tried ) { tried = true; char const * fn = getenv("DACC_EMUL_TRAV"); if ( fn ) f = fopen(fn,"w"); } return f; }
 #define FSTAT_MX(i,x) g_fstats.mx(i,x)
 #define FSTAT_ADD(i,x) g_fstats.add(i,x)
+#define FTRAV_EVENT(...) { FILE * const tf_ = ftrav_file(); if ( tf_ ) fprintf(tf_,__VA_ARGS__); }
 struct FeasIters { std::vector<uint32_t> it, ln; void clear() { it.clear(); ln.clear(); } };
 static FeasIters g_feasit;
 static inline void feasit_dump()
@@ -148,6 +149,7 @@
 #define FEAS_OVER() over(128);
 #define FSTAT_MX(i,x)
 #define FSTAT_ADD(i,x)
+#define FTRAV_EVENT(...) {}
 #endif
 }
 #endif
diff --git a/daccord_amd/csrc/fast_layout.hpp b/daccord_amd/csrc/fast_layout.hpp
--- a/daccord_amd/csrc/fast_layout.hpp
+++ b/daccord_amd/csrc/fast_layout.hpp
@@ -12,6 +12,7 @@
 
 HDEV constexpr uint32_t fcpow2(uint32_t v) { uint32_t p = 1; while ( p < v ) p <<= 1; return p; }
 HDEV constexpr uint32_t fcmax(uint32_t a, uint32_t b) { return a > b ? a : b; }
+HDEV constexpr uint32_t fcpad8(uint32_t v) { return (v + 7u) & ~7u; }
 template<bool W, typename A, typename B> struct FWideSel { typedef A type; };
 template<typename A, typename B> struct FWideSel<false,A,B> { typedef B type; };
 
@@ -19,6 +20,21 @@
 	static constexpr uint32_t o_##name = (start); \
 	static constexpr uint32_t e_##name = (o_##name + static_cast<uint32_t>(sizeof(type))*static_cast<uint32_t>(count) + 7u) & ~7u; \
 	HDEV LDSQ type * name() const { return reinterpret_cast<LDSQ type *>(base + o_##name); }
+
+struct FPE { uint32_t parent, stretch, pos, len; };
+#define FPOOL(pfx,get,put,packed) \
+	HDEV FPE get(uint32_t const slot) const \
+	{ \
+		FPE e; \
+		if constexpr ( packed ) { uint32_t const w = pfx##ent()[slot]; e.parent = w & 0xFFu; e.stretch = (w >> 8) & 0xFFu; e.pos = (w >> 16) & 0xFFu; e.len = w >> 24; } \
+		else { e.parent = pfx##parent()[slot]; e.stretch = pfx##stretch()[slot]; e.pos = pfx##pos()[slot]; e.len = pfx##len()[slot]; } \
+		return e; \
+	} \
+	HDEV void put(uint32_t const slot, uint32_t const pl, uint32_t const stretch, uint32_t const pos) const \
+	{ \
+		if constexpr ( packed ) pfx##ent()[slot] = pl | (stretch << 8) | (pos << 16); \
+		else { pfx##parent()[slot] = pl; pfx##stretch()[slot] = stretch; pfx##len()[slot] = pl >> 24; pfx##pos()[slot] = pos; }       \
+	}
 
 template<typename CT, bool GW = (CT::gw != 0)> struct FastLds;
 
@@ -116,12 +132,15 @@
 	FLD(siq,FSI,CT::siqcap,e_cseq)
 	static_assert(sizeof(FSI)*CT::siqcap <= lscrbytes,"the serial score interval heap shares the lane scratch");
 	static constexpr uint32_t pbase = fcmax(e_consL,e_lscr);
+	static constexpr bool pent = false;
 	FLD(rc_w,uint64_t,CT::rccap,pbase)
-	FLD(rc_parent,typename CT::id_t,CT::rccap,e_rc_w)
+	FLD(rc_ent,uint32_t,0,e_rc_w)
+	FLD(rc_parent,typename CT::id_t,CT::rccap,e_rc_ent)
 	FLD(rc_stretch,uint8_t,CT::rccap,e_rc_parent)
 	FLD(rc_pos,uint8_t,CT::rccap,e_rc_stretch)
 	FLD(rc_len,uint8_t,CT::rccap,e_rc_pos)
 	FLD(rc_baselen,uint8_t,CT::rccap,e_rc_len)
+	FPOOL(rc_,rcGet,rcPut,false)
 	FLD(rc_acc,typename CT::id_t,CT::rccap,e_rc_baselen)
 	FLD(rc_ord,typename CT::id_t,CT::rccap,e_rc_acc)
 	FLD(rc_arw,typename CT::id_t,CT::rccap,e_rc_ord)
@@ -133,16 +152,18 @@
 	FLD(rtmask,uint64_t,CT::fnc+1,e_rmaxw)
 	FLD(rfmask,uint64_t,CT::fnc+1,e_rtmask)
 	FLD(f_w,uint64_t,CT::fcap,e_rfmask)
-	FLD(f_parent,typename CT::id_t,CT::fcap,e_f_w)
+	FLD(f_ent,uint32_t,0,e_f_w)
+	FLD(f_parent,typename CT::id_t,CT::fcap,e_f_ent)
 	FLD(f_stretch,uint8_t,CT::fcap,e_f_parent)
 	FLD(f_pos,uint8_t,CT::fcap,e_f_stretch)
 	FLD(f_baselen,uint8_t,CT::fcap,e_f_pos)
 	FLD(f_len,uint8_t,CT::fcap,e_f_baselen)
+	FPOOL(f_,fGet,fPut,pent)
 	FLD(fp_id,typename CT::id_t,CT::fcap,e_f_len)
-	FLD(fp_cl,uint8_t,CT::fcap,e_fp_id)
-	FLD(fp_front,uint32_t,CT::fcap,e_fp_cl)
+	FLD(fp_front,uint32_t,CT::fcap,e_fp_id)
 	FLD(fp_adj,uint64_t,CT::fcap,e_fp_front)
-	FLD(fchb,uint8_t,8*CT::fnw*(CT::fnc+1),e_fp_adj)
+	FLD(f_free,uint8_t,fcpad8(CT::fcap),e_fp_adj)
+	FLD(fchb,uint8_t,8*CT::fnw*(CT::fnc+1),e_f_free)
 	FLD(fnp,uint16_t,CT::fnc+1,e_fchb)
 	FLD(ffm,uint64_t,CT::fnc+1,e_fnp)
 	FLD(ftm,uint64_t,CT::fnc+1,e_ffm)
@@ -249,12 +270,15 @@
 	FLD(mlast,uint64_t,keycap,e_mfirst)
 	static constexpr uint32_t send = (e_mlast + 15u) & ~15u;
 	static constexpr uint32_t sbytes = send - sbase;
+	static constexpr bool pent = sizeof(typename CT::id_t) == 1 && sizeof(sid_t) == 1;
 	FLD(rc_w,uint64_t,CT::rccap,sbase)
-	FLD(rc_parent,typename CT::id_t,CT::rccap,e_rc_w)
+	FLD(rc_ent,uint32_t,0,e_rc_w)
+	FLD(rc_parent,typename CT::id_t,CT::rccap,e_rc_ent)
 	FLD(rc_stretch,sid_t,CT::rccap,e_rc_parent)
 	FLD(rc_pos,uint8_t,CT::rccap,e_rc_stretch)
 	FLD(rc_len,uint8_t,CT::rccap,e_rc_pos)
 	FLD(rc_baselen,uint8_t,CT::rccap,e_rc_len)
+	FPOOL(rc_,rcGet,rcPut,false)
 	FLD(rc_acc,typename CT::id_t,CT::rccap,e_rc_baselen)
 	FLD(rc_ord,typename CT::id_t,CT::rccap,e_rc_acc)
 	FLD(rc_arw,typename CT::id_t,CT::rccap,e_rc_ord)
@@ -266,16 +290,18 @@
 	FLD(rtmask,uint64_t,CT::fnc+1,e_rmaxw)
 	FLD(rfmask,uint64_t,CT::fnc+1,e_rtmask)
 	FLD(f_w,uint64_t,CT::fcap,e_rfmask)
-	FLD(f_parent,typename CT::id_t,CT::fcap,e_f_w)
-	FLD(f_stretch,sid_t,CT::fcap,e_f_parent)
-	FLD(f_pos,uint8_t,CT::fcap,e_f_stretch)
+	FLD(f_ent,uint32_t,(pent ? CT::fcap : 0u),e_f_w)
+	FLD(f_parent,typename CT::id_t,(pent ? 0u : CT::fcap),e_f_ent)
+	FLD(f_stretch,sid_t,(pent ? 0u : CT::fcap),e_f_parent)
+	FLD(f_pos,uint8_t,(pent ? 0u : CT::fcap),e_f_stretch)
 	FLD(f_baselen,uint8_t,CT::fcap,e_f_pos)
-	FLD(f_len,uint8_t,CT::fcap,e_f_baselen)
+	FLD(f_len,uint8_t,(pent ? 0u : CT::fcap),e_f_baselen)
+	FPOOL(f_,fGet,fPut,pent)
 	FLD(fp_id,typename CT::id_t,CT::fcap,e_f_len)
-	FLD(fp_cl,uint8_t,CT::fcap,e_fp_id)
-	FLD(fp_front,uint32_t,CT::fcap,e_fp_cl)
+	FLD(fp_front,uint32_t,CT::fcap,e_fp_id)
 	FLD(fp_adj,uint64_t,CT::fcap,e_fp_front)
-	FLD(fchb,uint8_t,8*CT::fnw*(CT::fnc+1),e_fp_adj)
+	FLD(f_free,uint8_t,(pent ? 5u*fcpad8(CT::fcap) - fcpad8(4u*CT::fcap) : fcpad8(CT::fcap)),e_fp_adj)
+	FLD(fchb,uint8_t,8*CT::fnw*(CT::fnc+1),e_f_free)
 	FLD(fnp,uint16_t,CT::fnc+1,e_fchb)
 	FLD(ffm,uint64_t,CT::fnc+1,e_fnp)
 	FLD(ftm,uint64_t,CT::fnc+1,e_ffm)
@@ -372,6 +398,7 @@
 	static_assert(!oneslab || CT::gmem != 0,"a one-slab tier is a device-memory tier");
 };
 #undef FLD
+#undef FPOOL
 
 template<typename CT>
 HDEV FastCaps fastCapsOf(uint32_t const nrows, uint32_t const nsup)
diff --git a/daccord_amd/csrc/fast_window.hpp b/daccord_amd/csrc/fast_window.hpp
--- a/daccord_amd/csrc/fast_window.hpp
+++ b/daccord_amd/csrc/fast_window.hpp
@@ -1913,19 +1913,19 @@
 			return 64u*wd + static_cast<uint32_t>(__builtin_ctzll(m));
 		}
 	}
-	DEV int32_t extendPath(FEnum & F, uint32_t const parent, uint32_t const s, uint32_t const ppos, uint32_t const plen, uint64_t const pw, uint32_t const pbl,
+	DEV int32_t extendPath(FEnum & F, uint32_t const pl, uint32_t const s, uint32_t const ppos, uint64_t const pw, uint32_t const pbl,
 		int32_t const sfo, uint64_t const wf, uint64_t const wf1, uint32_t & npos, uint32_t & nbl, uint64_t & nw)
 	{
 		uint32_t const slot = clEnsure<FCH>(F.C,F.np,L.ctr()+1,CT::fcap/FCH);
 		if ( slot == ~0u ) { over(512|0x10000); return -1; }
 		uint32_t const slen = L.sslen()[s];
 		uint64_t weight = pw; uint32_t baselen = pbl;
-		if ( plen == 0 ) { baselen = slen+k-1; weight = sfo >= 0 ? wf : 0; }
+		if ( (pl >> 24) == 1 ) { baselen = slen+k-1; weight = sfo >= 0 ? wf : 0; }
 		else { baselen += slen-1; if ( sfo >= 0 ) weight += wf - wf1; }
 		npos = ppos + (slen-1); nbl = baselen; nw = weight;
-		if ( baselen > FBLMAX || npos > 255 || plen+1 > 255 ) { over(2048); return -1; }
+		if ( baselen > FBLMAX || npos > 255 || (pl >> 24) == 0 ) { over(2048); return -1; }
 		++F.np;
-		L.f_parent()[slot] = parent; L.f_stretch()[slot] = s; L.f_len()[slot] = plen+1; L.f_pos()[slot] = npos;
+		L.fPut(slot,pl,s,npos);
 		L.f_w()[slot] = weight; L.f_baselen()[slot] = baselen;
 		return slot;
 	}
@@ -1942,7 +1942,7 @@
 				int32_t const sfo = sfFind(sx,0);
 				uint64_t const wf = sfo >= 0 ? wuF(sfo) : 0;
 				uint32_t npos, nbl; uint64_t nw;
-				int32_t const id = extendPath(F,0,sx,0,0,0,0,sfo,wf,0,npos,nbl,nw);
+				int32_t const id = extendPath(F,1u << 24,sx,0,0,0,sfo,wf,0,npos,nbl,nw);
 				if ( id < 0 ) return;
 				if constexpr ( CT::wide == 0 ) { if ( nbl < 64 ) F.m0 |= 1ull << nbl; else F.m1 |= 1ull << (nbl-64); } else fblSet(F,nbl);
 			}
@@ -1958,6 +1958,7 @@
 				if ( zz < 64 ) F.m0 &= F.m0-1; else F.m1 &= F.m1-1;
 			}
 			else zz = fblPop(F);
+			if ( zz >= 64 ) FTRAV_EVENT("TZ %d %u\n",int(CT::maxs),zz)
 			uint32_t hn = 0;
 			for ( uint32_t i0 = 0; i0 < F.np; i0 += 64 )
 			{
@@ -1968,8 +1969,10 @@
 				{
 					uint32_t const slot = clSlot<FCH>(F.C,i0+i);
 					uint32_t const b4 = *reinterpret_cast<LDSQ uint32_t const *>(L.f_baselen() + slot);
-					#pragma unroll
-					for ( uint32_t u = 0; u < 4; ++u ) if ( i+u < ie ) mem |= static_cast<uint64_t>(((b4 >> (8*u)) & 0xFF) == zz) << (i+u);
+					uint32_t const rem = ie-i;
+					uint32_t const q4 = dacc_eq4n(b4,zz,rem);
+					mem |= static_cast<uint64_t>(q4) << i;
+					if ( q4 && rem < 4 ) FTRAV_EVENT("TG %d %u %u\n",int(CT::maxs),zz,rem)
 				}
 				SITE(12)
 				while ( mem )
@@ -1989,22 +1992,23 @@
 			{
 				uint32_t const path = hp[0];
 				ipop<true>(hp,hn,W);
-				uint32_t const ps = L.f_stretch()[path], ppos = L.f_pos()[path], plen = L.f_len()[path], pbl = zz;
+				FPE const pe = L.fGet(path);
+				uint32_t const ps = pe.stretch, ppos = pe.pos, plen = pe.len, pbl = zz;
 				uint64_t const pw = W[path];
 				uint32_t const lastn = L.slast()[ps];
 				SITE(14)
 				{
 					int32_t const psfo = sfFind(ps,ppos - (L.sslen()[ps]-1));
 					uint32_t const pfront = L.nv()[lastn];
-					uint32_t const o = clSlot<FCH>(F.C,F.nfpop);
-					L.fp_id()[o] = path; L.fp_front()[o] = pfront; L.fp_cl()[o] = ppos; F.ffm |= 1ull << (pfront & 63);
-					L.fp_adj()[o] = psfo >= 0 ? (pw - recF(psfo).wl) : pw;
+					L.fp_id()[clSlot<FCH>(F.C,F.nfpop)] = path; L.fp_front()[path] = pfront; F.ffm |= 1ull << (pfront & 63);
+					L.fp_adj()[path] = psfo >= 0 ? (pw - recF(psfo).wl) : pw;
 					if ( pw > F.fmaxw ) F.fmaxw = pw;
 					++F.nfpop;
 				}
 				SITE(15)
 				if ( pbl < k || ( static_cast<int64_t>(pbl-k) < ((lmax+1)/2) ) )
 				{
+					uint32_t const pl = path | ((plen+1) << 24);
 					MIt it; byFirstBegin(V,it,lastn);
 					for ( int32_t sx = byFirstNext(V,it); sx >= 0; sx = byFirstNext(V,it) )
 					{
@@ -2015,7 +2019,7 @@
 						if ( eweight >= FW_THRES_01 )
 						{
 							uint32_t npos, nbl; uint64_t nw;
-							int32_t const ep = extendPath(F,path,s,ppos,plen,pw,pbl,sfo,eweight,fr.w1,npos,nbl,nw);
+							int32_t const ep = extendPath(F,pl,s,ppos,pw,pbl,sfo,eweight,fr.w1,npos,nbl,nw);
 							if ( ep < 0 ) return;
 							if ( nw >= FW_THRES_01 && static_cast<int64_t>(npos) + k <= lmax )
 							{
@@ -2039,7 +2043,7 @@
 		{
 			uint32_t const path = L.fp_id()[clSlot<FCH>(F.C,i)];
 			uint32_t const pbl = L.f_baselen()[path];
-			if ( pbl < k || ( static_cast<int64_t>(pbl-k) < ((lmax+1)/2) ) ) m |= 1ull << (L.slast()[L.f_stretch()[path]] & 63);
+			if ( pbl < k || ( static_cast<int64_t>(pbl-k) < ((lmax+1)/2) ) ) m |= 1ull << (L.slast()[L.fGet(path).stretch] & 63);
 		}
 		L.fnp()[fi] = F.nfpop; L.ffm()[fi] = F.ffm; L.ftm()[fi] = m; L.fmx()[fi] = F.fmaxw;
 	}
@@ -2054,7 +2058,7 @@
 			uint32_t const pbl = L.f_baselen()[path];
 			if ( pbl < k || ( static_cast<int64_t>(pbl-k) < ((lmax+1)/2) ) )
 			{
-				uint32_t const target = L.slast()[L.f_stretch()[path]];
+				uint32_t const target = L.slast()[L.fGet(path).stretch];
 				if ( target == pfirst || target == ln ) return false;
 			}
 		}
@@ -2066,15 +2070,16 @@
 	uint32_t cfree;
 	DEV uint32_t buildSeq(uint32_t const path, uint32_t const rp, LDSQ sid_t * dst, uint32_t & conslen)
 	{
-		uint32_t const nf = L.f_len()[path], nr = L.rc_len()[rp];
+		FPE ef = L.fGet(path);
+		uint32_t const nf = ef.len, nr = L.rc_len()[rp];
 		if ( nf + nr > FSEQCAP ) { over(4096); return ~0u; }
-		conslen = static_cast<uint32_t>(L.f_pos()[path]) + k + L.rc_pos()[rp];
+		conslen = ef.pos + k + L.rc_pos()[rp];
 		if ( conslen > CONSROW ) { over(4096); return ~0u; }
-		uint32_t qf = path, qr = rp;
+		uint32_t qr = rp;
 		uint32_t const ns = nf > nr ? nf : nr;
 		for ( uint32_t t = 0; t < ns; ++t )
 		{
-			if ( t < nf ) { dst[nf-1-t] = L.f_stretch()[qf]; qf = L.f_parent()[qf]; }
+			if ( t < nf ) { dst[nf-1-t] = ef.stretch; ef = L.fGet(ef.parent); }
 			if ( t < nr ) { dst[nf+t] = L.rc_stretch()[qr]; qr = L.rc_parent()[qr]; }
 		}
 		return nf+nr;
@@ -2138,8 +2143,9 @@
 		uint32_t qf = pb;
 		for ( uint32_t t = 0; t < d; ++t )
 		{
-			if ( L.f_stretch()[qf] != mid[d-1-t] ) return false;
-			qf = L.f_parent()[qf];
+			FPE const e = L.fGet(qf);
+			if ( e.stretch != mid[d-1-t] ) return false;
+			qf = e.parent;
 		}
 		return qf == pa;
 	}
@@ -2148,8 +2154,9 @@
 		FSTAT_ADD(18,1);
 		SITE_T0
 		if ( ncdh == 16 ) { uint32_t const to = L.cdh()[0].o, tl = L.cdh()[0].l; if ( !(tl & UNMAT) ) cfree |= 1u << to; spop<FCC,true>(L.cdh(),ncdh); SITE(5) }
-		uint32_t const nf = L.f_len()[path], nr = L.rc_len()[rp];
-		uint32_t const conslen = static_cast<uint32_t>(L.f_pos()[path]) + k + L.rc_pos()[rp];
+		FPE const ef = L.fGet(path);
+		uint32_t const nf = ef.len, nr = L.rc_len()[rp];
+		uint32_t const conslen = ef.pos + k + L.rc_pos()[rp];
 		if ( nf + nr > FSEQCAP || conslen > CONSROW ) { over(4096); return false; }
 		uint32_t const n = nf+nr;
 		SITE(6)
@@ -2216,14 +2223,14 @@
 		if ( !skip ) { pvpath = pvrp = pvnf = 0; pvcl = ~0u; }
 		for ( uint32_t pi = 0; pi < nfpop; ++pi )
 		{
-			uint32_t const o = clSlot<FCH>(FC,pi);
-			uint32_t const front = L.fp_front()[o];
+			uint32_t const path = L.fp_id()[clSlot<FCH>(FC,pi)];
+			uint32_t const front = L.fp_front()[path];
 			if ( !((rfm >> (front & 63)) & 1) ) continue;
 			uint32_t sub, sup, mi;
-			if ( scoreInterval(sbase,nacc2,front,static_cast<int64_t>(L.fp_cl()[o]) + k,lmin,lmax,sub,sup,mi) )
+			if ( scoreInterval(sbase,nacc2,front,static_cast<int64_t>(L.fGet(path).pos) + k,lmin,lmax,sub,sup,mi) )
 			{
 				if ( nsiq >= CT::siqcap ) { over(512|0x40000); return; }
-				FSI si; si.left = sub; si.right = sup; si.current = mi; si.path = pi; si.w = L.fp_adj()[o] + L.rc_w()[L.rc_ord()[sbase+mi]];
+				FSI si; si.left = sub; si.right = sup; si.current = mi; si.path = path; si.w = L.fp_adj()[path] + L.rc_w()[L.rc_ord()[sbase+mi]];
 				spush<FSI,false>(L.siq(),nsiq,si);
 			}
 		}
@@ -2235,20 +2242,20 @@
 			uint32_t bi;
 			if ( scoreNext(sbase,si.left,si.right,si.current,bi) )
 			{
-				FSI sic = si; sic.current = bi; sic.w = L.fp_adj()[clSlot<FCH>(FC,si.path)] + L.rc_w()[L.rc_ord()[sbase+bi]];
+				FSI sic = si; sic.current = bi; sic.w = L.fp_adj()[si.path] + L.rc_w()[L.rc_ord()[sbase+bi]];
 				if ( nsiq >= CT::siqcap ) { over(512|0x40000); return; }
 				spush<FSI,false>(L.siq(),nsiq,sic);
 			}
 			if ( numfullpath < skip ) continue;
-			if ( !offerCandidate(si.w,L.fp_id()[clSlot<FCH>(FC,si.path)],L.rc_ord()[sbase+si.current],pn) ) return;
+			if ( !offerCandidate(si.w,si.path,L.rc_ord()[sbase+si.current],pn) ) return;
 		}
 	}
 	struct PSI { id_t path, current, left, right; };
 	enum { PSIQ = CT::psiq, POUTE = 8 };
-	static constexpr id_t PSENT = static_cast<id_t>(~static_cast<id_t>(0));
-	static_assert(sizeof(id_t) > 1 || 8u*FNW*FCH < 255u,"the end mark of a lane's interval heap must not be a forward pop index");
+	DEV static void psiMark(LDSQ PSI * e) { e->right = 0; }
+	DEV static bool psiMarked(PSI const & e) { return e.right == 0; }
 	bool lscrdirty;
-	DEV uint64_t psiW(PSI const & e, ChunkList<FNW> const & FC, uint32_t const sbase) const { return L.fp_adj()[clSlot<FCH>(FC,e.path)] + L.rc_w()[L.rc_ord()[sbase+e.current]]; }
+	DEV uint64_t psiW(PSI const & e, uint32_t const sbase) const { return L.fp_adj()[e.path] + L.rc_w()[L.rc_ord()[sbase+e.current]]; }
 	DEV uint32_t combineLane(ChunkList<FNW> const & FC, uint32_t const nfpop, uint32_t const sbase, uint32_t const nacc2, uint64_t const rfm, int64_t const lmin, int64_t const lmax,
 		uint32_t const maxfullpath, LDSQ PSI * H, LDSQ id_t * out, bool const prune, uint64_t const T0)
 	{
@@ -2256,21 +2263,21 @@
 		SITE_T0
 		for ( uint32_t pi = 0; pi < nfpop; ++pi )
 		{
-			uint32_t const o = clSlot<FCH>(FC,pi);
-			uint32_t const front = L.fp_front()[o];
+			uint32_t const path = L.fp_id()[clSlot<FCH>(FC,pi)];
+			uint32_t const front = L.fp_front()[path];
 			if ( !((rfm >> (front & 63)) & 1) ) continue;
 			uint32_t sub, sup, mi;
-			if ( scoreInterval(sbase,nacc2,front,static_cast<int64_t>(L.fp_cl()[o]) + k,lmin,lmax,sub,sup,mi) )
+			if ( scoreInterval(sbase,nacc2,front,static_cast<int64_t>(L.fGet(path).pos) + k,lmin,lmax,sub,sup,mi) )
 			{
 				if ( n >= PSIQ || sup > 255 && sizeof(id_t) == 1 ) return 0xFF;
-				PSI e; e.path = pi; e.current = mi; e.left = sub; e.right = sup;
+				PSI e; e.path = path; e.current = mi; e.left = sub; e.right = sup;
 				uint32_t i = n++; H[i] = e;
-				uint64_t const we = psiW(e,FC,sbase);
+				uint64_t const we = psiW(e,sbase);
 				while ( i )
 				{
 					uint32_t const p = (i-1)>>1;
 					PSI const ep = H[p];
-					if ( we > psiW(ep,FC,sbase) ) { H[i] = ep; H[p] = e; i = p; }
+					if ( we > psiW(ep,sbase) ) { H[i] = ep; H[p] = e; i = p; }
 					else break;
 				}
 			}
@@ -2286,22 +2293,22 @@
 		for ( uint32_t numfullpath = 0; n && numfullpath < maxfullpath; ++numfullpath )
 		{
 			PSI const top = H[0];
-			if ( prune && psiW(top,FC,sbase) <= T0 ) { if ( n < PSIQ ) H[n].path = PSENT; return cnt | 0x20; }
-			if ( cnt == POUTE ) { if ( n < PSIQ ) H[n].path = PSENT; return cnt | 0x10; }
+			if ( prune && psiW(top,sbase) <= T0 ) { if ( n < PSIQ ) psiMark(H+n); return cnt | 0x20; }
+			if ( cnt == POUTE ) { if ( n < PSIQ ) psiMark(H+n); return cnt | 0x10; }
 			{
 				--n; PSI const last = H[n]; H[0] = last;
 				uint32_t i = 0, r;
 				while ( (r = 2*i+2) < n )
 				{
-					uint32_t const m = psiW(H[r-1],FC,sbase) > psiW(H[r],FC,sbase) ? (r-1) : r;
+					uint32_t const m = psiW(H[r-1],sbase) > psiW(H[r],sbase) ? (r-1) : r;
 					PSI const em = H[m], ei = H[i];
-					if ( psiW(ei,FC,sbase) > psiW(em,FC,sbase) ) break;
+					if ( psiW(ei,sbase) > psiW(em,sbase) ) break;
 					H[i] = em; H[m] = ei; i = m;
 				}
 				if ( r >= n )
 				{
 					uint32_t const l = 2*i+1;
-					if ( l < n ) { PSI const el = H[l], ei = H[i]; if ( !(psiW(ei,FC,sbase) > psiW(el,FC,sbase)) ) { H[i] = el; H[l] = ei; } }
+					if ( l < n ) { PSI const el = H[l], ei = H[i]; if ( !(psiW(ei,sbase) > psiW(el,sbase)) ) { H[i] = el; H[l] = ei; } }
 				}
 			}
 			uint32_t bi;
@@ -2309,16 +2316,16 @@
 			{
 				PSI e = top; e.current = bi;
 				uint32_t i = n++; H[i] = e;
-				uint64_t const we = psiW(e,FC,sbase);
+				uint64_t const we = psiW(e,sbase);
 				while ( i )
 				{
 					uint32_t const p = (i-1)>>1;
 					PSI const ep = H[p];
-					if ( we > psiW(ep,FC,sbase) ) { H[i] = ep; H[p] = e; i = p; }
+					if ( we > psiW(ep,sbase) ) { H[i] = ep; H[p] = e; i = p; }
 					else break;
 				}
 			}
-			out[2*cnt] = static_cast<id_t>(clSlot<FCH>(FC,top.path)); out[2*cnt+1] = L.rc_ord()[sbase+top.current]; ++cnt;
+			out[2*cnt] = top.path; out[2*cnt+1] = L.rc_ord()[sbase+top.current]; ++cnt;
 			SITE(2)
 		}
 		return cnt;
@@ -2328,25 +2335,25 @@
 		uint32_t nm = 0;
 		for ( uint32_t pi = 0; pi < nfpop; ++pi )
 		{
-			uint32_t const front = L.fp_front()[clSlot<FCH>(FC,pi)];
+			uint32_t const path = L.fp_id()[clSlot<FCH>(FC,pi)];
+			uint32_t const front = L.fp_front()[path];
 			if ( !((rfm >> (front & 63)) & 1) ) continue;
-			if ( nm < PSIQ ) H[nm].path = static_cast<id_t>(pi);
+			if ( nm < PSIQ ) H[nm].path = static_cast<id_t>(path);
 			++nm;
 		}
 		return nm;
 	}
 	DEV bool intervalTask(ChunkList<FNW> const & FC, uint32_t const sbase, uint32_t const nacc2, int64_t const lmin, int64_t const lmax, LDSQ PSI * e) const
 	{
-		uint32_t const pi = e->path;
-		uint32_t const o = clSlot<FCH>(FC,pi);
+		uint32_t const path = e->path;
 		uint32_t sub, sup, mi;
-		if ( scoreInterval(sbase,nacc2,L.fp_front()[o],static_cast<int64_t>(L.fp_cl()[o]) + k,lmin,lmax,sub,sup,mi) )
+		if ( scoreInterval(sbase,nacc2,L.fp_front()[path],static_cast<int64_t>(L.fGet(path).pos) + k,lmin,lmax,sub,sup,mi) )
 		{
 			if ( sup > 255 && sizeof(id_t) == 1 ) return false;
-			PSI v; v.path = static_cast<id_t>(pi); v.current = static_cast<id_t>(mi); v.left = static_cast<id_t>(sub); v.right = static_cast<id_t>(sup);
+			PSI v; v.path = static_cast<id_t>(path); v.current = static_cast<id_t>(mi); v.left = static_cast<id_t>(sub); v.right = static_cast<id_t>(sup);
 			*e = v;
 		}
-		else e->path = PSENT;
+		else psiMark(e);
 		return true;
 	}
 	DEV uint32_t heapOfList(ChunkList<FNW> const & FC, uint32_t const sbase, LDSQ PSI * H, uint32_t const nm) const
@@ -2355,14 +2362,14 @@
 		for ( uint32_t j = 0; j < nm; ++j )
 		{
 			PSI const e = H[j];
-			if ( e.path == PSENT ) continue;
+			if ( psiMarked(e) ) continue;
 			uint32_t i = n++; H[i] = e;
-			uint64_t const we = psiW(e,FC,sbase);
+			uint64_t const we = psiW(e,sbase);
 			while ( i )
 			{
 				uint32_t const p = (i-1)>>1;
 				PSI const ep = H[p];
-				if ( we > psiW(ep,FC,sbase) ) { H[i] = ep; H[p] = e; i = p; }
+				if ( we > psiW(ep,sbase) ) { H[i] = ep; H[p] = e; i = p; }
 				else break;
 			}
 		}
@@ -2375,11 +2382,10 @@
 		SITE_T0
 		for ( uint32_t e = 0; e < cnt; ++e )
 		{
-			uint32_t const o = out[2*e];
+			uint32_t const fid = out[2*e];
 			uint32_t const rp = out[2*e+1];
-			uint64_t const w = L.fp_adj()[o] + L.rc_w()[rp];
+			uint64_t const w = L.fp_adj()[fid] + L.rc_w()[rp];
 			if ( ncdh == 16 && w <= L.cdh()[0].w ) { if ( e == 0 ) FSTAT_ADD(20,1); SITE(4) return false; }
-			uint32_t const fid = L.fp_id()[o];
 			SITE(4)
 			if ( !offerCandidate(w,fid,rp,pn) ) return false;
 			SITE_RESET
@@ -2390,26 +2396,26 @@
 	DEV void continueLane(ChunkList<FNW> const & FC, uint32_t const sbase, LDSQ PSI * H, uint32_t const cnt, uint32_t pn)
 	{
 		uint32_t n = 0;
-		while ( n < PSIQ && H[n].path != PSENT ) ++n;
+		while ( n < PSIQ && !psiMarked(H[n]) ) ++n;
 		for ( uint32_t numfullpath = cnt; n && numfullpath < 16; ++numfullpath )
 		{
 			PSI const top = H[0];
-			uint64_t const wtop = psiW(top,FC,sbase);
+			uint64_t const wtop = psiW(top,sbase);
 			if ( ncdh == 16 && wtop <= L.cdh()[0].w ) break;
 			{
 				--n; PSI const last = H[n]; H[0] = last;
 				uint32_t i = 0, r;
 				while ( (r = 2*i+2) < n )
 				{
-					uint32_t const m = psiW(H[r-1],FC,sbase) > psiW(H[r],FC,sbase) ? (r-1) : r;
+					uint32_t const m = psiW(H[r-1],sbase) > psiW(H[r],sbase) ? (r-1) : r;
 					PSI const em = H[m], ei = H[i];
-					if ( psiW(ei,FC,sbase) > psiW(em,FC,sbase) ) break;
+					if ( psiW(ei,sbase) > psiW(em,sbase) ) break;
 					H[i] = em; H[m] = ei; i = m;
 				}
 				if ( r >= n )
 				{
 					uint32_t const l = 2*i+1;
-					if ( l < n ) { PSI const el = H[l], ei = H[i]; if ( !(psiW(ei,FC,sbase) > psiW(el,FC,sbase)) ) { H[i] = el; H[l] = ei; } }
+					if ( l < n ) { PSI const el = H[l], ei = H[i]; if ( !(psiW(ei,sbase) > psiW(el,sbase)) ) { H[i] = el; H[l] = ei; } }
 				}
 			}
 			uint32_t bi;
@@ -2417,16 +2423,16 @@
 			{
 				PSI e = top; e.current = bi;
 				uint32_t i = n++; H[i] = e;
-				uint64_t const we = psiW(e,FC,sbase);
+				uint64_t const we = psiW(e,sbase);
 				while ( i )
 				{
 					uint32_t const p = (i-1)>>1;
 					PSI const ep = H[p];
-					if ( we > psiW(ep,FC,sbase) ) { H[i] = ep; H[p] = e; i = p; }
+					if ( we > psiW(ep,sbase) ) { H[i] = ep; H[p] = e; i = p; }
 					else break;
 				}
 			}
-			if ( !offerCandidate(wtop,L.fp_id()[clSlot<FCH>(FC,top.path)],L.rc_ord()[sbase+top.current],pn) ) return;
+			if ( !offerCandidate(wtop,top.path,L.rc_ord()[sbase+top.current],pn) ) return;
 		}
 	}
 
@@ -2751,16 +2757,17 @@
 					if ( used && ( (mode & 0x10) || ((mode & 0x20) && !(ncdh == 16 && L.cdh()[0].w >= roundT0)) ) )
 					{
 						pcount(21,1);
+						FTRAV_EVENT("TP %d %c\n",int(CT::maxs),lscrdirty ? 's' : 'c')
 						if ( !lscrdirty ) continueLane(FC,L.rbase()[li],reinterpret_cast<LDSQ PSI *>(L.lscr()) + PSIQ*q,cnt,pn);
 						else combinePair(FC,L.fnp()[fi],L.rbase()[li],L.rn()[li],L.rfmask()[li],lmin,lmax,16,cnt,pn);
 						SITE(9)
 					}
 				}
-				else { pcount(23,1); lscrdirty = true; combinePair(FC,L.fnp()[fi],L.rbase()[li],L.rn()[li],L.rfmask()[li],lmin,lmax,16); SITE(9) }
+				else { pcount(23,1); FTRAV_EVENT("TP %d s\n",int(CT::maxs)) lscrdirty = true; combinePair(FC,L.fnp()[fi],L.rbase()[li],L.rn()[li],L.rfmask()[li],lmin,lmax,16); SITE(9) }
 				if ( flags ) return 0;
 				continue;
 			}
-			pcount(22,1);
+			pcount(22,1); FTRAV_EVENT("TP %d x\n",int(CT::maxs))
 			lscrdirty = true;
 			bool const rcached = mode & 1, fcached = mode & 2, same = mode & 4;
 			uint32_t const sf = L.parF()[fi], sl = L.parL()[li];
diff --git a/daccord_amd/csrc/wave.hpp b/daccord_amd/csrc/wave.hpp
--- a/daccord_amd/csrc/wave.hpp
+++ b/daccord_amd/csrc/wave.hpp
@@ -377,6 +377,13 @@
 	x &= 0xFFFFu; x = (x | (x << 8)) & 0x00FF00FFu; x = (x | (x << 4)) & 0x0F0F0F0Fu; x = (x | (x << 2)) & 0x33333333u; x = (x | (x << 1)) & 0x55555555u;
 	return x;
 }
+HDEV uint32_t dacc_eq4(uint32_t const b4, uint32_t const z)
+{
+	uint32_t const x = b4 ^ (z * 0x01010101u);
+	uint32_t const m = ~(((x & 0x7F7F7F7Fu) + 0x7F7F7F7Fu) | x | 0x7F7F7F7Fu);
+	return ((m >> 7) | (m >> 14) | (m >> 21) | (m >> 28)) & 0xFu;
+}
+HDEV uint32_t dacc_eq4n(uint32_t const b4, uint32_t const z, uint32_t const n) { return dacc_eq4(b4,z) & (n < 4 ? (1u << n)-1u : 0xFu); }
 HDEV uint32_t next_pow2(uint32_t v)
 {
 	uint32_t p = 1;
```

New measurement: 42.60. No clear change (-0.1%).
